# snarkify/sirius

Hardware: AMD Instinct MI355X
Metric: IVC fold-steps/s (CycleFold IVC::next hot path, Poseidon-shaped synthetic trace, 2^k rows) (higher is better)
Workload: dtype u256 (modular; 9 x 29-bit / 8 x 32-bit limbs)

## Files before the change

sirius_amd/csrc/msm.h:

```cpp
#pragma once
#include "curve.cuh"
#include "devrt.h"
#include "glv.cuh"
#include "stripes.h"
#include "tuning.h"

#include <cstdlib>

namespace srs {
namespace msm {

constexpr int WBITS = 16;
constexpr int NWIN = 16;
constexpr int NWIN_COMPACT = 8;
constexpr uint32_t PAY_ENDO = 1u << 30;
constexpr uint32_t NBUCKET = 1u << (WBITS - 1);

constexpr uint32_t SORT_THREADS = 1024;
constexpr uint32_t SORT_TILE_MIN = 8192;
constexpr uint32_t SORT_TARGET_BLOCKS = 256;
constexpr uint32_t SEG = 128, SEG_BUCKETS = NBUCKET / SEG;
constexpr uint32_t SORT_TILE2 = 8192;
constexpr uint64_t TWO_PASS_MIN_SLOTS = 1ull << 23;
constexpr uint32_t PLAN_THREADS = 1024;
constexpr uint32_t ACC_THREADS = 256;
constexpr uint32_t ACC_L0_LOG = 4, ACC_L0 = 1u << ACC_L0_LOG;
constexpr uint32_t ACC_L1_LOG = 3, ACC_L1 = 1u << ACC_L1_LOG;
constexpr uint32_t FINAL_THREADS = 256;
constexpr uint32_t FINAL_FANIN = 512;
constexpr int MAX_LEVELS = 8;
constexpr uint32_t RED_ROWS = 256;
constexpr uint32_t RED_COLS = NBUCKET / RED_ROWS;
constexpr uint32_t RED_THREADS = 4 * RED_COLS;
constexpr uint32_t ACC1_QUAD_MAX = 1u << 17;
constexpr uint32_t BATCH_ARGS = 16;
constexpr uint32_t LANDING_SLOTS = 16;
constexpr uint32_t NORM_G = 16;
constexpr uint32_t SLOT_LOG = 6;
constexpr uint32_t SLOT_L0_MIN_LOG = 2, SLOT_L0_MAX_LOG = 16;
constexpr int WBITS_W = 20;
constexpr int NWIN_W = 13;
constexpr uint32_t NSEG_W = 16;
constexpr uint32_t WIDE_THREADS = 256, WIDE_PER = 2, WIDE_TILE = WIDE_THREADS * WIDE_PER;
constexpr uint32_t WIDE_MIN_KEY_LOG = 23;
constexpr uint32_t WIDE_MIN_N_LOG = 23;

static_assert(RED_ROWS == 256 && RED_COLS == 128, "k_rowcol lane layout");
static_assert(NBUCKET % PLAN_THREADS == 0, "k_plan tiling");

inline bool expect_ovf_initial() { return tuning::get_or(tuning::MSM_EXPECT_OVF, 1) != 0; }

struct Key {
    int curve = 0;
    size_t len = 0;
    size_t global_len = 0;
    uint32_t rank = 0, world = 1;
    bool compact = false;
    bool compact_scalars = false;
    affine_t *table = nullptr;
    affine_t *table_w = nullptr;
    uint64_t stat_slot_sets = 0, stat_hot_sets = 0, stat_redo = 0, stat_other_sets = 0;
    uint64_t last_entries = 0;
    uint64_t last_scalars = 0;

    Arena arena;
    void *h_result = nullptr;
    struct Landing { bool wide = false, slot_mode = false, ovf_on = false; uint32_t batch = 0; } landing[LANDING_SLOTS];
    xyzz_t *fold_buckets = nullptr;
    xyzz_t *slots = nullptr;
    size_t slots_pts = 0;
    uint8_t *used = nullptr;
    uint32_t *h_ovf = nullptr;
    uint32_t slot_s = 0;
    uint32_t seq = 0;
    bool commit_ovf = false;
    bool expect_ovf = expect_ovf_initial();
    uint32_t cold_streak = 0;
};

int choose_windows(Key &k);
void build_table(Key &k, hipStream_t stream);
size_t table_bytes(const Key &k);
void release(Key &k);
void generate_bases(Key &k, uint64_t seed, hipStream_t stream);

void read_bases(const Key &k, affine_t *out_dev, hipStream_t stream);

size_t count_off_curve(const Key &k, hipStream_t stream);

size_t workspace_bytes(uint32_t n_max, uint32_t batch);

void run(Key &k, const fe_t *const *scalars_dev, const uint32_t *n_host, uint32_t batch, int is_mont,
         hipStream_t stream, xyzz_t *result_host);

enum Fold { FOLD_NONE = 0, FOLD_FIRST = 1, FOLD_MIDDLE = 2, FOLD_LAST = 3 };
bool enqueue(Key &k, const fe_t *const *scalars_dev, const uint32_t *n_host, const uint32_t *base_host, uint32_t batch, int is_mont,
             hipStream_t stream, uint32_t slot, Fold fold = FOLD_NONE);
void finish(Key &k, uint32_t batch, uint32_t slot, bool launched, xyzz_t *result_host);
void reserve(Key &k, uint32_t n_max, uint32_t batch);
bool overflow_missed(const Key &k, uint32_t slot);
void note_commit(Key &k, const uint32_t *slots_used, uint32_t n_slots, uint64_t scalars);

}
}
```

sirius_amd/csrc/msm.hip:

```cpp
#define SRS_F29_CHAIN 1
#include "msm.h"
#include "tuning.h"
#include "curve29.cuh"
#include "prof.h"

#include <algorithm>
#include <cstdlib>
#include <numeric>
#include <vector>

namespace srs {
namespace msm {

__device__ __forceinline__ uint32_t upper_bucket(const uint32_t *__restrict__ tp, uint32_t t) {
    uint32_t lo = 0, hi = NBUCKET;
    while (hi - lo > 1) {
        uint32_t mid = (lo + hi) >> 1;
        if (tp[mid] <= t) lo = mid; else hi = mid;
    }
    return lo;
}

template <class C>
__global__ void k_table_step(const affine_t *__restrict__ prev, xyzz_t *__restrict__ tmp, uint32_t n, int nbits) {
    uint32_t i = blockIdx.x * blockDim.x + threadIdx.x;
    if (i >= n) return;
    affine_t p = prev[i];
    xyzz_t a;
    if (Ec<C>::is_identity(p)) {
        a = Ec<C>::identity();
    } else {
        a = Ec<C>::dbl_affine(p);
        for (int k = 1; k < nbits; ++k) a = Ec<C>::dbl(a);
    }
    tmp[i] = a;
}

template <class C>
__global__ void k_normalize(const xyzz_t *__restrict__ in, affine_t *__restrict__ out, uint32_t n) {
    using F = typename C::F;
    uint32_t g = blockIdx.x * blockDim.x + threadIdx.x;
    size_t lo = (size_t)g * NORM_G;
    if (lo >= n) return;
    uint32_t cnt = (uint32_t)((n - lo < NORM_G) ? (n - lo) : NORM_G);
    fe_t pre[NORM_G];
    fe_t acc = F::one();
    for (uint32_t j = 0; j < cnt; ++j) {
        pre[j] = acc;
        xyzz_t p = in[lo + j];
        if (!Ec<C>::is_identity(p)) acc = F::mul(acc, F::mul(p.zz, p.zzz));
    }
    fe_t inv = F::inv(acc);
    for (uint32_t j = cnt; j-- > 0;) {
        xyzz_t p = in[lo + j];
        affine_t o;
        if (Ec<C>::is_identity(p)) {
            o = Ec<C>::affine_identity();
        } else {
            fe_t i = F::mul(inv, pre[j]);
            inv = F::mul(inv, F::mul(p.zz, p.zzz));
            o.x = F::mul(p.x, F::mul(i, p.zzz));
            o.y = F::mul(p.y, F::mul(i, p.zz));
        }
        out[lo + j] = o;
    }
}

template <class C>
__global__ void k_table_form(affine_t *__restrict__ t, size_t n) {
    size_t i = (size_t)blockIdx.x * blockDim.x + threadIdx.x;
    if (i >= n) return;
    t[i] = Ec29<C>::table_form(t[i]);
}
template <class C>
__device__ __forceinline__ affine_t table_unform(const affine_t &q) {
    using G = typename C::F;
    fe_t c = G::one();
    for (int d = 0; d < 5; ++d) c = G::halve(c);
    affine_t o;
    o.x = G::mul(q.x, c);
    o.y = G::mul(q.y, c);
    return o;
}
template <class C>
__global__ void k_table_unform(const affine_t *__restrict__ t, affine_t *__restrict__ out, size_t n) {
    size_t i = (size_t)blockIdx.x * blockDim.x + threadIdx.x;
    if (i >= n) return;
    out[i] = table_unform<C>(t[i]);
}

__device__ __forceinline__ uint64_t splitmix64(uint64_t &s) {
    uint64_t z = (s += 0x9e3779b97f4a7c15ull);
    z = (z ^ (z >> 30)) * 0xbf58476d1ce4e5b9ull;
    z = (z ^ (z >> 27)) * 0x94d049bb133111ebull;
    return z ^ (z >> 31);
}
template <class C>
__global__ void k_gen_bases(xyzz_t *__restrict__ tmp, uint32_t n, uint64_t seed, uint32_t rank, uint32_t world) {
    using F = typename C::F;
    uint32_t i = blockIdx.x * blockDim.x + threadIdx.x;
    if (i >= n) return;
    uint64_t g = Stripes{rank, world}.global_index((size_t)i);
    uint64_t st = seed ^ (g * 0x100000001b3ull + 0xcbf29ce484222325ull);
    uint32_t k[8];
    for (int j = 0; j < 4; ++j) {
        uint64_t v = splitmix64(st);
        k[2 * j] = (uint32_t)v;
        k[2 * j + 1] = (uint32_t)(v >> 32);
    }
    k[7] &= 0x0FFFFFFFu;
    k[0] |= 1u;
    affine_t gen;
    gen.x = F::one();
    if (C::ID == 0) {
        gen.y = F::dbl(F::one());
    } else {
        fe_t y;
        const uint32_t yc[8] = {0x823f272cu, 0x833fc48du, 0xf1181294u, 0x2d270d45u, 0x06a45d63u, 0xcf135e75u, 0x00000002u, 0u};
        for (int j = 0; j < 8; ++j) y.v[j] = yc[j];
        gen.y = F::to_mont(y);
    }
    tmp[i] = Ec<C>::mul_canon(k, gen);
}

template <class C>
__global__ void k_on_curve(const affine_t *__restrict__ pts, uint32_t n, uint32_t *__restrict__ bad) {
    uint32_t i = blockIdx.x * blockDim.x + threadIdx.x;
    if (i >= n) return;
    if (!Ec<C>::is_on_curve(table_unform<C>(pts[i]))) atomicAdd(bad, 1u);
}

struct BatchDesc {
    const fe_t *ptr[BATCH_ARGS];
    uint32_t n[BATCH_ARGS];
    uint32_t base[BATCH_ARGS];
};

__device__ __forceinline__ void recode_half(const uint32_t (&k)[4], bool neg, uint16_t *__restrict__ d, size_t n) {
    const uint32_t top = neg ? 0x7FFFu : 0x8000u;
    uint32_t carry = 0;
#pragma unroll
    for (int w = 0; w < NWIN_COMPACT; ++w) {
        const uint32_t v = ((k[w >> 1] >> ((w & 1) * 16)) & 0xFFFFu) + carry;
        const bool borrow = v > top;
        const uint32_t mag = borrow ? 0x10000u - v : v;
        const bool minus = borrow != neg;
        carry = borrow ? 1u : 0u;
        d[(size_t)w * n] = (uint16_t)(mag ? ((mag - 1u) | (minus ? 0x8000u : 0u)) : 0xFFFFu);
    }
}

template <class C, bool COMPACT>
__global__ void k_digits(BatchDesc bd, uint16_t *__restrict__ dig, size_t dig_stride, int is_mont, uint32_t rank, uint32_t world,
                         uint32_t *__restrict__ count_zero, uint32_t n_zero) {
    using S = typename C::S;
    uint32_t m = blockIdx.y;
    uint32_t n = bd.n[m];
    uint32_t i = blockIdx.x * blockDim.x + threadIdx.x;
    for (uint32_t j = (blockIdx.y * gridDim.x + blockIdx.x) * blockDim.x + threadIdx.x; j < n_zero; j += gridDim.x * gridDim.y * blockDim.x)
        count_zero[j] = 0;
    if (i >= n) return;
    fe_t s = bd.ptr[m][Stripes{rank, world}.global_index((size_t)i)];
    if (is_mont) s = S::from_mont(s);
    uint16_t *d = dig + (size_t)m * dig_stride;
    if (COMPACT) {
        const glv_t g = glv_decompose<C>(s);
        recode_half(g.k1, g.neg1, d + i, n);
        recode_half(g.k2, g.neg2, d + (size_t)NWIN_COMPACT * n + i, n);
        return;
    }
    uint32_t carry = 0;
#pragma unroll
    for (int w = 0; w < NWIN; ++w) {
        uint32_t raw = (s.v[w >> 1] >> ((w & 1) * 16)) & 0xFFFFu;
        uint32_t v = raw + carry;
        uint32_t code;
        if (v > 0x8000u) {
            code = ((0x10000u - v) - 1u) | 0x8000u;
            carry = 1;
        } else {
            code = v ? (v - 1u) : 0xFFFFu;
            carry = 0;
        }
        d[(size_t)w * n + i] = (uint16_t)code;
    }
}

template <class Fn>
__device__ __forceinline__ void for_each_digit(const uint16_t *__restrict__ d, uint32_t lo, uint32_t hi, Fn fn) {
    uint32_t head = lo;
    while (head < hi && (reinterpret_cast<uintptr_t>(d + head) & 15u)) ++head;
    for (uint32_t i = lo + threadIdx.x; i < head; i += blockDim.x) fn(i, (uint32_t)d[i]);
    const uint32_t nvec = (hi - head) / 8;
    const uint4 *v = reinterpret_cast<const uint4 *>(d + head);
    auto eight = [&](uint32_t q, const uint4 &x) {
        const uint32_t i0 = head + q * 8;
        fn(i0 + 0, x.x & 0xFFFFu); fn(i0 + 1, x.x >> 16);
        fn(i0 + 2, x.y & 0xFFFFu); fn(i0 + 3, x.y >> 16);
        fn(i0 + 4, x.z & 0xFFFFu); fn(i0 + 5, x.z >> 16);
        fn(i0 + 6, x.w & 0xFFFFu); fn(i0 + 7, x.w >> 16);
    };
    uint32_t q = threadIdx.x;
    for (; q + 3 * blockDim.x < nvec; q += 4 * blockDim.x) {
        const uint4 x0 = v[q], x1 = v[q + blockDim.x], x2 = v[q + 2 * blockDim.x], x3 = v[q + 3 * blockDim.x];
        eight(q, x0); eight(q + blockDim.x, x1); eight(q + 2 * blockDim.x, x2); eight(q + 3 * blockDim.x, x3);
    }
    for (; q < nvec; q += blockDim.x) eight(q, v[q]);
    for (uint32_t i = head + nvec * 8 + threadIdx.x; i < hi; i += blockDim.x) fn(i, (uint32_t)d[i]);
}

__device__ __forceinline__ void tile_histogram(uint32_t *h, const uint16_t *__restrict__ d, uint32_t lo, uint32_t hi) {
    for (uint32_t b = threadIdx.x; b < NBUCKET; b += blockDim.x) h[b] = 0;
    __syncthreads();
    for_each_digit(d, lo, hi, [&](uint32_t, uint32_t code) {
        if (code != 0xFFFFu) atomicAdd(&h[code & 0x7FFFu], 1u);
    });
    __syncthreads();
}

__global__ void SRS_KERNEL_BOUNDS(SORT_THREADS, 1)
    k_hist(const uint16_t *__restrict__ dig, size_t dig_stride, BatchDesc bd,
           uint32_t *__restrict__ count , uint32_t SORT_TILE,
           uint32_t *__restrict__ tile_hist ) {
    __shared__ uint32_t h[NBUCKET];
    uint32_t m = blockIdx.z, w = blockIdx.y;
    uint32_t n = bd.n[m];
    uint32_t lo = blockIdx.x * SORT_TILE;
    const uint32_t T1 = gridDim.x * NWIN, t1 = w * gridDim.x + blockIdx.x;
    if (lo >= n) {
        if (tile_hist)
            for (uint32_t sgm = threadIdx.x; sgm < SEG; sgm += blockDim.x) tile_hist[((size_t)m * SEG + sgm) * T1 + t1] = 0;
        return;
    }
    uint32_t hi = lo + SORT_TILE < n ? lo + SORT_TILE : n;
    const uint16_t *d = dig + (size_t)m * dig_stride + (size_t)w * n;
    tile_histogram(h, d, lo, hi);
    uint32_t *cnt = count + (size_t)m * NBUCKET;
    const uint32_t rot = ((blockIdx.y * gridDim.x + blockIdx.x) * 128u) & (NBUCKET - 1);
    for (uint32_t i = threadIdx.x; i < NBUCKET; i += blockDim.x) {
        const uint32_t b = (i + rot) & (NBUCKET - 1);
        uint32_t c = h[b];
        if (c) atomicAdd(&cnt[b], c);
    }
    if (tile_hist) {
        for (uint32_t sgm = threadIdx.x; sgm < SEG; sgm += blockDim.x) {
            uint32_t c = 0;
            for (uint32_t b = 0; b < SEG_BUCKETS; ++b) c += h[sgm * SEG_BUCKETS + ((b + sgm) & (SEG_BUCKETS - 1))];
            tile_hist[((size_t)m * SEG + sgm) * T1 + t1] = c;
        }
    }
}

__device__ __forceinline__ uint32_t block_exclusive_scan(uint32_t v, uint32_t *lds, uint32_t *total);

__global__ void SRS_KERNEL_BOUNDS(1024, 1)
    k_scan_seg(uint32_t *__restrict__ tile_hist, uint32_t T1, const uint32_t *__restrict__ plan, size_t plan_stride) {
    __shared__ uint32_t lds[64];
    const uint32_t sgm = blockIdx.x, m = blockIdx.y;
    uint32_t *row = tile_hist + ((size_t)m * SEG + sgm) * T1;
    const uint32_t base = plan[(size_t)m * plan_stride + (size_t)sgm * SEG_BUCKETS];
    uint32_t carry = 0;
    for (uint32_t at = 0; at < T1; at += blockDim.x) {
        const uint32_t i = at + threadIdx.x;
        const uint32_t v = i < T1 ? row[i] : 0;
        uint32_t total;
        const uint32_t ex = block_exclusive_scan(v, lds, &total);
        if (i < T1) row[i] = base + carry + ex;
        carry += total;
    }
}

constexpr uint32_t GRP_PER = 16, GRP_SUB = SORT_THREADS * GRP_PER;
template <bool COMPACT>
__device__ __forceinline__ uint32_t payload_base(uint32_t w, uint32_t table_stride, uint32_t base) {
    if (COMPACT) return ((w & (NWIN_COMPACT - 1)) * table_stride + base) | (w >= NWIN_COMPACT ? PAY_ENDO : 0u);
    return w * table_stride + base;
}
template <bool COMPACT>
__global__ void SRS_KERNEL_BOUNDS(SORT_THREADS, 1)
    k_group(const uint16_t *__restrict__ dig, size_t dig_stride, BatchDesc bd, const uint32_t *__restrict__ tile_hist,
            uint16_t *__restrict__ gkey, uint32_t *__restrict__ gpay, size_t g_stride, uint32_t table_stride, uint32_t SORT_TILE,
            const uint32_t *__restrict__ plan, size_t plan_stride, uint16_t *__restrict__ tb, size_t tb_stride, uint32_t arr) {
    __shared__ uint32_t cur[SEG], cnt[SEG], lb[SEG], sc[64];
    __shared__ uint32_t spay[GRP_SUB];
    __shared__ uint16_t skey[GRP_SUB];
    const uint32_t m = blockIdx.z, w = blockIdx.y, tid = threadIdx.x;
    if (tb) {
        const uint32_t *tp = plan + (size_t)m * plan_stride + (size_t)arr * (NBUCKET + 1);
        uint16_t *map = tb + (size_t)m * tb_stride;
        const uint32_t waves = gridDim.x * gridDim.y * (blockDim.x >> 6);
        const uint32_t wv = (blockIdx.y * gridDim.x + blockIdx.x) * (blockDim.x >> 6) + (tid >> 6), lane = tid & 63u;
        for (uint32_t b = wv; b < NBUCKET; b += waves) {
            const uint32_t s = tp[b], e = tp[b + 1];
            for (uint32_t t = s + lane; t < e; t += 64) map[t] = (uint16_t)b;
        }
    }
    const uint32_t n = bd.n[m];
    const uint32_t lo = blockIdx.x * SORT_TILE;
    if (lo >= n) return;
    const uint32_t hi = lo + SORT_TILE < n ? lo + SORT_TILE : n;
    const uint32_t T1 = gridDim.x * NWIN, t1 = w * gridDim.x + blockIdx.x;
    for (uint32_t sgm = tid; sgm < SEG; sgm += blockDim.x) cur[sgm] = tile_hist[((size_t)m * SEG + sgm) * T1 + t1];
    const uint16_t *d = dig + (size_t)m * dig_stride + (size_t)w * n;
    uint16_t *ok = gkey + (size_t)m * g_stride;
    uint32_t *op = gpay + (size_t)m * g_stride;
    const uint32_t pay0 = payload_base<COMPACT>(w, table_stride, bd.base[m]);
    for (uint32_t sub = lo; sub < hi; sub += GRP_SUB) {
        for (uint32_t sgm = tid; sgm < SEG; sgm += blockDim.x) cnt[sgm] = 0;
        __syncthreads();
        const uint32_t i0 = sub + tid * GRP_PER;
        uint32_t code[GRP_PER], rank[GRP_PER];
        if (i0 + GRP_PER <= hi && (reinterpret_cast<uintptr_t>(d + i0) & 15u) == 0) {
            const uint4 *v = reinterpret_cast<const uint4 *>(d + i0);
#pragma unroll
            for (uint32_t q = 0; q < GRP_PER / 8; ++q) {
                const uint4 x = v[q];
                code[8 * q + 0] = x.x & 0xFFFFu; code[8 * q + 1] = x.x >> 16;
                code[8 * q + 2] = x.y & 0xFFFFu; code[8 * q + 3] = x.y >> 16;
                code[8 * q + 4] = x.z & 0xFFFFu; code[8 * q + 5] = x.z >> 16;
                code[8 * q + 6] = x.w & 0xFFFFu; code[8 * q + 7] = x.w >> 16;
            }
        } else {
#pragma unroll
            for (uint32_t k = 0; k < GRP_PER; ++k) code[k] = i0 + k < hi ? (uint32_t)d[i0 + k] : 0xFFFFu;
        }
#pragma unroll
        for (uint32_t k = 0; k < GRP_PER; ++k)
            rank[k] = code[k] != 0xFFFFu ? atomicAdd(&cnt[(code[k] & 0x7FFFu) / SEG_BUCKETS], 1u) : 0u;
        __syncthreads();
        uint32_t n_sub;
        const uint32_t ex = block_exclusive_scan(tid < SEG ? cnt[tid] : 0u, sc, &n_sub);
        if (tid < SEG) lb[tid] = ex;
        __syncthreads();
#pragma unroll
        for (uint32_t k = 0; k < GRP_PER; ++k) {
            if (code[k] != 0xFFFFu) {
                const uint32_t bkt = code[k] & 0x7FFFu, pos = lb[bkt / SEG_BUCKETS] + rank[k];
                skey[pos] = (uint16_t)bkt;
                spay[pos] = (pay0 + i0 + k) | ((code[k] & 0x8000u) << 16);
            }
        }
        __syncthreads();
        for (uint32_t i = tid; i < n_sub; i += blockDim.x) {
            const uint32_t key = skey[i], sgm = key / SEG_BUCKETS, g = cur[sgm] + (i - lb[sgm]);
            ok[g] = (uint16_t)key;
            op[g] = spay[i];
        }
        __syncthreads();
        if (tid < SEG) cur[tid] += cnt[tid];
    }
}

constexpr uint32_t S2_PER = 8, S2_RANGE = 2 * SEG_BUCKETS;
static_assert(SORT_TILE2 == SORT_THREADS * S2_PER, "k_scatter2: one tile = S2_PER entries per thread");
__global__ void SRS_KERNEL_BOUNDS(SORT_THREADS, 2)
    k_scatter2(const uint16_t *__restrict__ gkey, const uint32_t *__restrict__ gpay, size_t g_stride,
               const uint32_t *__restrict__ plan, size_t plan_stride, uint32_t *__restrict__ cursor ,
               uint32_t *__restrict__ sorted, size_t sorted_stride, uint32_t TILE2) {
    __shared__ uint32_t cnt[S2_RANGE], lb[S2_RANGE], gb[S2_RANGE], sc[64];
    __shared__ uint32_t spay[SORT_TILE2];
    __shared__ uint16_t skey[SORT_TILE2];
    const uint32_t m = blockIdx.y, tid = threadIdx.x;
    const uint32_t total = plan[(size_t)m * plan_stride + NBUCKET];
    const uint32_t n_tiles = (total + TILE2 - 1) / TILE2, per_xcd = (n_tiles + 7) / 8;
    if (blockIdx.x / 8 >= per_xcd) return;
    const uint32_t tile_id = (blockIdx.x % 8) * per_xcd + blockIdx.x / 8;
    if (tile_id >= n_tiles) return;
    const uint32_t lo = tile_id * TILE2;
    if (lo >= total) return;
    const uint32_t hi = lo + TILE2 < total ? lo + TILE2 : total;
    const uint16_t *key = gkey + (size_t)m * g_stride;
    const uint32_t *pay = gpay + (size_t)m * g_stride;
    uint32_t *cur = cursor + (size_t)m * NBUCKET;
    uint32_t *out = sorted + (size_t)m * sorted_stride;
    const uint32_t b_lo = ((uint32_t)key[lo] / SEG_BUCKETS) * SEG_BUCKETS;
    const uint32_t b_hi = ((uint32_t)key[hi - 1] / SEG_BUCKETS + 1) * SEG_BUCKETS;
    if (b_hi - b_lo > S2_RANGE) {
        for (uint32_t i = lo + tid; i < hi; i += blockDim.x) out[atomicAdd(&cur[key[i]], 1u)] = pay[i];
        return;
    }
    for (uint32_t b = tid; b < S2_RANGE; b += blockDim.x) cnt[b] = 0;
    __syncthreads();
    const uint32_t i0 = lo + tid * S2_PER;
    uint32_t kk[S2_PER], pp[S2_PER], rank[S2_PER];
    if (i0 + S2_PER <= hi && (reinterpret_cast<uintptr_t>(key + i0) & 15u) == 0 && (reinterpret_cast<uintptr_t>(pay + i0) & 15u) == 0) {
        const uint4 x = *reinterpret_cast<const uint4 *>(key + i0);
        kk[0] = x.x & 0xFFFFu; kk[1] = x.x >> 16; kk[2] = x.y & 0xFFFFu; kk[3] = x.y >> 16;
        kk[4] = x.z & 0xFFFFu; kk[5] = x.z >> 16; kk[6] = x.w & 0xFFFFu; kk[7] = x.w >> 16;
        const uint4 p0 = *reinterpret_cast<const uint4 *>(pay + i0), p1 = *reinterpret_cast<const uint4 *>(pay + i0 + 4);
        pp[0] = p0.x; pp[1] = p0.y; pp[2] = p0.z; pp[3] = p0.w; pp[4] = p1.x; pp[5] = p1.y; pp[6] = p1.z; pp[7] = p1.w;
    } else {
#pragma unroll
        for (uint32_t k = 0; k < S2_PER; ++k) {
            kk[k] = i0 + k < hi ? (uint32_t)key[i0 + k] : 0xFFFFu;
            pp[k] = i0 + k < hi ? pay[i0 + k] : 0u;
        }
    }
#pragma unroll
    for (uint32_t k = 0; k < S2_PER; ++k) rank[k] = kk[k] != 0xFFFFu ? atomicAdd(&cnt[kk[k] - b_lo], 1u) : 0u;
    __syncthreads();
    uint32_t n_tile;
    const uint32_t c = tid < S2_RANGE ? cnt[tid] : 0u;
    const uint32_t ex = block_exclusive_scan(c, sc, &n_tile);
    if (tid < S2_RANGE) {
        lb[tid] = ex;
        gb[tid] = c ? atomicAdd(&cur[b_lo + tid], c) : 0u;
    }
    __syncthreads();
#pragma unroll
    for (uint32_t k = 0; k < S2_PER; ++k) {
        if (kk[k] != 0xFFFFu) {
            const uint32_t pos = lb[kk[k] - b_lo] + rank[k];
            skey[pos] = (uint16_t)(kk[k] - b_lo);
            spay[pos] = pp[k];
        }
    }
    __syncthreads();
    for (uint32_t i = tid; i < n_tile; i += blockDim.x) {
        const uint32_t b = skey[i];
        out[gb[b] + (i - lb[b])] = spay[i];
    }
}

#ifndef SCATTER_RES_INFLIGHT
#define SCATTER_RES_INFLIGHT 4
#endif
template <bool COMPACT>
__global__ void SRS_KERNEL_BOUNDS(SORT_THREADS, 1)
    k_scatter(const uint16_t *__restrict__ dig, size_t dig_stride, BatchDesc bd,
              uint32_t *__restrict__ cursor , uint32_t *__restrict__ sorted,
              size_t sorted_stride, uint32_t table_stride, uint32_t SORT_TILE) {
    __shared__ uint32_t h[NBUCKET];
    uint32_t m = blockIdx.z, w = blockIdx.y;
    uint32_t n = bd.n[m];
    uint32_t lo = blockIdx.x * SORT_TILE;
    if (lo >= n) return;
    uint32_t hi = lo + SORT_TILE < n ? lo + SORT_TILE : n;
    const uint16_t *d = dig + (size_t)m * dig_stride + (size_t)w * n;
    tile_histogram(h, d, lo, hi);
    uint32_t *cur = cursor + (size_t)m * NBUCKET;
    constexpr int RES = SCATTER_RES_INFLIGHT;
    for (uint32_t b0 = threadIdx.x; b0 < NBUCKET; b0 += RES * blockDim.x) {
        uint32_t c[RES], r[RES];
#pragma unroll
        for (int u = 0; u < RES; ++u) c[u] = b0 + u * blockDim.x < NBUCKET ? h[b0 + u * blockDim.x] : 0u;
#pragma unroll
        for (int u = 0; u < RES; ++u) r[u] = c[u] ? atomicAdd(&cur[b0 + u * blockDim.x], c[u]) : 0u;
#pragma unroll
        for (int u = 0; u < RES; ++u) if (c[u]) h[b0 + u * blockDim.x] = r[u];
    }
    __syncthreads();
    uint32_t *out = sorted + (size_t)m * sorted_stride;
    const uint32_t pay0 = payload_base<COMPACT>(w, table_stride, bd.base[m]);
    for_each_digit(d, lo, hi, [&](uint32_t i, uint32_t code) {
        if (code != 0xFFFFu) {
            uint32_t pos = atomicAdd(&h[code & 0x7FFFu], 1u);
            out[pos] = (pay0 + i) | ((code & 0x8000u) << 16);
        }
    });
}

struct Link {
    uint32_t base[MAX_LEVELS + 1][NSEG_W + 1];
};
__device__ __forceinline__ uint32_t link_segment(const uint32_t *__restrict__ base, uint32_t t) {
    uint32_t v = 0;
#pragma unroll
    for (uint32_t u = 1; u < NSEG_W; ++u) v += (t >= base[u]) ? 1u : 0u;
    return v;
}

struct WideDesc {
    const fe_t *ptr;
    uint32_t n, base;
    uint32_t rank, world;
    int is_mont;
};

template <class C>
__device__ __forceinline__ void wide_codes(const WideDesc &wd, uint32_t i, uint32_t (&code)[NWIN_W]) {
    using S = typename C::S;
    if (i >= wd.n) {
#pragma unroll
        for (int w = 0; w < NWIN_W; ++w) code[w] = 0xFFFFFFFFu;
        return;
    }
    fe_t s = wd.ptr[Stripes{wd.rank, wd.world}.global_index((size_t)i)];
    if (wd.is_mont) s = S::from_mont(s);
    uint32_t carry = 0;
#pragma unroll
    for (int w = 0; w < NWIN_W; ++w) {
        const int bit = WBITS_W * w, limb = bit >> 5, sh = bit & 31;
        uint64_t two = s.v[limb];
        if (limb + 1 < 8) two |= (uint64_t)s.v[limb + 1] << 32;
        const uint32_t v = ((uint32_t)(two >> sh) & 0xFFFFFu) + carry;
        if (v > 0x80000u) {
            code[w] = ((0x100000u - v) - 1u) | 0x80000000u;
            carry = 1;
        } else {
            code[w] = v ? (v - 1u) : 0xFFFFFFFFu;
            carry = 0;
        }
    }
}

template <class C, bool GROUP>
__global__ void SRS_KERNEL_BOUNDS(WIDE_THREADS, 1)
    k_seg_pass(WideDesc wd, uint32_t *__restrict__ tile_cnt, uint32_t T, uint32_t *__restrict__ seg_total,
               uint16_t *__restrict__ gkey, uint32_t *__restrict__ gpay, uint32_t table_stride) {
    constexpr uint32_t NW = WIDE_THREADS / 64, STAGE = GROUP ? WIDE_TILE * NWIN_W : 1;
    __shared__ uint32_t wc[NW][NSEG_W];
    __shared__ uint32_t ss[NSEG_W + 1], goff[NSEG_W];
    __shared__ uint16_t skey[STAGE];
    __shared__ uint32_t spay[STAGE];
    const uint32_t tile = blockIdx.x, wave = threadIdx.x >> 6;
    if (threadIdx.x < NW * NSEG_W) (&wc[0][0])[threadIdx.x] = 0;
    uint32_t code[WIDE_PER][NWIN_W];
#pragma unroll
    for (uint32_t k = 0; k < WIDE_PER; ++k) wide_codes<C>(wd, tile * WIDE_TILE + k * WIDE_THREADS + threadIdx.x, code[k]);
    __syncthreads();
#pragma unroll
    for (uint32_t k = 0; k < WIDE_PER; ++k) {
#pragma unroll
        for (int w = 0; w < NWIN_W; ++w) {
            const uint32_t c = code[k][w];
            if (c != 0xFFFFFFFFu) atomicAdd(&wc[wave][(c >> 15) & (NSEG_W - 1)], 1u);
        }
    }
    __syncthreads();
    if (threadIdx.x < NSEG_W) {
        const uint32_t v = threadIdx.x;
        uint32_t tot = 0;
        for (uint32_t w = 0; w < NW; ++w) tot += wc[w][v];
        if (!GROUP) {
            tile_cnt[(size_t)v * T + tile] = tot;
            if (tot) atomicAdd(&seg_total[v], tot);
        } else {
            ss[v + 1] = tot;
            goff[v] = tile_cnt[(size_t)v * T + tile];
        }
    }
    if (!GROUP) return;
    __syncthreads();
    if (threadIdx.x == 0) {
        uint32_t run = 0;
        for (uint32_t v = 0; v < NSEG_W; ++v) {
            const uint32_t c = ss[v + 1];
            ss[v] = run;
            run += c;
        }
        ss[NSEG_W] = run;
    }
    __syncthreads();
    if (threadIdx.x < NSEG_W) {
        const uint32_t v = threadIdx.x;
        uint32_t run = ss[v];
        for (uint32_t w = 0; w < NW; ++w) {
            const uint32_t c = wc[w][v];
            wc[w][v] = run;
            run += c;
        }
    }
    __syncthreads();
#pragma unroll
    for (uint32_t k = 0; k < WIDE_PER; ++k) {
        const uint32_t i = tile * WIDE_TILE + k * WIDE_THREADS + threadIdx.x;
#pragma unroll
        for (int w = 0; w < NWIN_W; ++w) {
            const uint32_t c = code[k][w];
            if (c != 0xFFFFFFFFu) {
                const uint32_t pos = atomicAdd(&wc[wave][(c >> 15) & (NSEG_W - 1)], 1u);
                skey[pos] = (uint16_t)(c & 0x7FFFu);
                spay[pos] = ((uint32_t)w * table_stride + wd.base + i) | (c & 0x80000000u);
            }
        }
    }
    __syncthreads();
    for (uint32_t v = 0; v < NSEG_W; ++v) {
        const uint32_t lo = ss[v], hi = ss[v + 1], g0 = goff[v];
        for (uint32_t e = lo + threadIdx.x; e < hi; e += WIDE_THREADS) {
            gkey[g0 + (e - lo)] = skey[e];
            gpay[g0 + (e - lo)] = spay[e];
        }
    }
}

__global__ void SRS_KERNEL_BOUNDS(1024, 1)
    k_seg_scan(uint32_t *__restrict__ tile_cnt, uint32_t T, const uint32_t *__restrict__ seg_total, uint32_t *__restrict__ seg_off,
               uint32_t *__restrict__ tile_base ,
               uint32_t *__restrict__ tile_base2 ,
               uint32_t small_tiles ) {
    __shared__ uint32_t lds[64];
    const uint32_t v = blockIdx.x;
    uint32_t base = 0;
    for (uint32_t u = 0; u < v; ++u) base += seg_total[u];
    if (v == 0 && threadIdx.x == 0) {
        uint32_t all = 0;
        for (uint32_t u = 0; u < NSEG_W; ++u) all += seg_total[u];
        uint32_t tile_g = (all + (SORT_TARGET_BLOCKS - NSEG_W) - 1) / (SORT_TARGET_BLOCKS - NSEG_W);
        tile_g = (tile_g + 1023u) & ~1023u;
        if (tile_g < SORT_TILE_MIN) tile_g = SORT_TILE_MIN;
        tile_base[NSEG_W + 1] = tile_g;
        uint32_t run = 0, tr = 0;
        for (uint32_t u = 0; u < NSEG_W; ++u) {
            seg_off[u] = run;
            tile_base[u] = tr;
            run += seg_total[u];
            tr += (seg_total[u] + tile_g - 1) / tile_g;
        }
        seg_off[NSEG_W] = run;
        tile_base[NSEG_W] = tr;
        const uint32_t tile2 = (small_tiles && all / (NSEG_W * NBUCKET) < 40u) ? SORT_TILE2 / 4 : SORT_TILE2;
        uint32_t t2 = 0;
        for (uint32_t u = 0; u < NSEG_W; ++u) {
            tile_base2[u] = t2;
            t2 += (seg_total[u] + tile2 - 1) / tile2;
        }
        tile_base2[NSEG_W] = t2;
        tile_base2[NSEG_W + 1] = tile2;
    }
    uint32_t *row = tile_cnt + (size_t)v * T;
    uint32_t carry = 0;
    for (uint32_t at = 0; at < T; at += blockDim.x) {
        const uint32_t i = at + threadIdx.x;
        const uint32_t c = i < T ? row[i] : 0;
        uint32_t total;
        const uint32_t ex = block_exclusive_scan(c, lds, &total);
        if (i < T) row[i] = base + carry + ex;
        carry += total;
    }
}

__device__ __forceinline__ bool wide_tile(const uint32_t *__restrict__ seg_off, const uint32_t *__restrict__ tile_base,
                                          uint32_t &v, uint32_t &lo, uint32_t &hi) {
    if (blockIdx.x >= tile_base[NSEG_W]) return false;
    const uint32_t tile_g = tile_base[NSEG_W + 1];
    v = link_segment(tile_base, blockIdx.x);
    lo = seg_off[v] + (blockIdx.x - tile_base[v]) * tile_g;
    hi = seg_off[v + 1];
    if (hi > lo + tile_g) hi = lo + tile_g;
    return true;
}

__global__ void SRS_KERNEL_BOUNDS(SORT_THREADS, 1)
    k_hist_g(const uint16_t *__restrict__ gkey, const uint32_t *__restrict__ seg_off, const uint32_t *__restrict__ tile_base,
             uint32_t *__restrict__ count , uint32_t *__restrict__ tile_hist ) {
    __shared__ uint32_t h[NBUCKET];
    uint32_t v, lo, hi;
    if (!wide_tile(seg_off, tile_base, v, lo, hi)) return;
    tile_histogram(h, gkey, lo, hi);
    uint32_t *cnt = count + (size_t)v * NBUCKET;
    for (uint32_t b = threadIdx.x; b < NBUCKET; b += blockDim.x) {
        uint32_t c = h[b];
        if (c) atomicAdd(&cnt[b], c);
    }
    if (tile_hist) {
        for (uint32_t sgm = threadIdx.x; sgm < SEG; sgm += blockDim.x) {
            uint32_t c = 0;
            for (uint32_t b = 0; b < SEG_BUCKETS; ++b) c += h[sgm * SEG_BUCKETS + ((b + sgm) & (SEG_BUCKETS - 1))];
            tile_hist[(size_t)sgm * gridDim.x + blockIdx.x] = c;
        }
    }
}

__global__ void SRS_KERNEL_BOUNDS(1024, 1)
    k_scan_seg_g(uint32_t *__restrict__ tile_hist, uint32_t TG, const uint32_t *__restrict__ tile_base, const uint32_t *__restrict__ plan,
                 size_t plan_stride) {
    __shared__ uint32_t lds[64];
    const uint32_t sgm = blockIdx.x, v = blockIdx.y;
    const uint32_t t0 = tile_base[v], t1 = tile_base[v + 1];
    uint32_t *row = tile_hist + (size_t)sgm * TG;
    const uint32_t base = plan[(size_t)v * plan_stride + (size_t)sgm * SEG_BUCKETS];
    uint32_t carry = 0;
    for (uint32_t at = t0; at < t1; at += blockDim.x) {
        const uint32_t i = at + threadIdx.x;
        const uint32_t c = i < t1 ? row[i] : 0;
        uint32_t total;
        const uint32_t ex = block_exclusive_scan(c, lds, &total);
        if (i < t1) row[i] = base + carry + ex;
        carry += total;
    }
}

__global__ void SRS_KERNEL_BOUNDS(SORT_THREADS, 1)
    k_group_g(const uint16_t *__restrict__ gkey, const uint32_t *__restrict__ gpay, const uint32_t *__restrict__ seg_off,
              const uint32_t *__restrict__ tile_base, const uint32_t *__restrict__ tile_hist, uint16_t *__restrict__ gkey2,
              uint32_t *__restrict__ gpay2) {
    __shared__ uint32_t cur[SEG], cnt[SEG], lb[SEG], sc[64];
    __shared__ uint32_t spay[GRP_SUB];
    __shared__ uint16_t skey[GRP_SUB];
    const uint32_t tid = threadIdx.x;
    uint32_t v, lo, hi;
    if (!wide_tile(seg_off, tile_base, v, lo, hi)) return;
    for (uint32_t sgm = tid; sgm < SEG; sgm += blockDim.x) cur[sgm] = tile_hist[(size_t)sgm * gridDim.x + blockIdx.x];
    for (uint32_t sub = lo; sub < hi; sub += GRP_SUB) {
        for (uint32_t sgm = tid; sgm < SEG; sgm += blockDim.x) cnt[sgm] = 0;
        __syncthreads();
        uint32_t key[GRP_PER], pay[GRP_PER], rank[GRP_PER];
#pragma unroll
        for (uint32_t k = 0; k < GRP_PER; ++k) {
            const uint32_t i = sub + k * SORT_THREADS + tid;
            key[k] = i < hi ? (uint32_t)gkey[i] : 0xFFFFu;
            pay[k] = i < hi ? gpay[i] : 0u;
        }
#pragma unroll
        for (uint32_t k = 0; k < GRP_PER; ++k) rank[k] = key[k] != 0xFFFFu ? atomicAdd(&cnt[key[k] / SEG_BUCKETS], 1u) : 0u;
        __syncthreads();
        uint32_t n_sub;
        const uint32_t ex = block_exclusive_scan(tid < SEG ? cnt[tid] : 0u, sc, &n_sub);
        if (tid < SEG) lb[tid] = ex;
        __syncthreads();
#pragma unroll
        for (uint32_t k = 0; k < GRP_PER; ++k) {
            if (key[k] != 0xFFFFu) {
                const uint32_t pos = lb[key[k] / SEG_BUCKETS] + rank[k];
                skey[pos] = (uint16_t)key[k];
                spay[pos] = pay[k];
            }
        }
        __syncthreads();
        for (uint32_t i = tid; i < n_sub; i += blockDim.x) {
            const uint32_t kk = skey[i], sgm = kk / SEG_BUCKETS, g = cur[sgm] + (i - lb[sgm]);
            gkey2[g] = (uint16_t)kk;
            gpay2[g] = spay[i];
        }
        __syncthreads();
        if (tid < SEG) cur[tid] += cnt[tid];
    }
}

__global__ void SRS_KERNEL_BOUNDS(SORT_THREADS, 2)
    k_scatter2_g(const uint16_t *__restrict__ gkey2, const uint32_t *__restrict__ gpay2, const uint32_t *__restrict__ seg_off,
                 const uint32_t *__restrict__ tile_base2, uint32_t *__restrict__ cursor ,
                 uint32_t *__restrict__ sorted) {
    __shared__ uint32_t cnt[S2_RANGE], lb[S2_RANGE], gb[S2_RANGE], sc[64];
    __shared__ uint32_t spay[SORT_TILE2];
    __shared__ uint16_t skey[SORT_TILE2];
    const uint32_t tid = threadIdx.x;
    const uint32_t n_tiles = tile_base2[NSEG_W], per_xcd = (n_tiles + 7) / 8;
    if (blockIdx.x / 8 >= per_xcd) return;
    const uint32_t tile_id = (blockIdx.x % 8) * per_xcd + blockIdx.x / 8;
    if (tile_id >= n_tiles) return;
    const uint32_t v = link_segment(tile_base2, tile_id), tile2 = tile_base2[NSEG_W + 1];
    const uint32_t lo = seg_off[v] + (tile_id - tile_base2[v]) * tile2;
    const uint32_t hi = lo + tile2 < seg_off[v + 1] ? lo + tile2 : seg_off[v + 1];
    if (lo >= hi) return;
    uint32_t *cur = cursor + (size_t)v * NBUCKET;
    const uint32_t b_lo = ((uint32_t)gkey2[lo] / SEG_BUCKETS) * SEG_BUCKETS;
    const uint32_t b_hi = ((uint32_t)gkey2[hi - 1] / SEG_BUCKETS + 1) * SEG_BUCKETS;
    if (b_hi - b_lo > S2_RANGE) {
        for (uint32_t i = lo + tid; i < hi; i += blockDim.x) sorted[atomicAdd(&cur[gkey2[i]], 1u)] = gpay2[i];
        return;
    }
    for (uint32_t b = tid; b < S2_RANGE; b += blockDim.x) cnt[b] = 0;
    __syncthreads();
    uint32_t kk[S2_PER], pp[S2_PER], rank[S2_PER];
#pragma unroll
    for (uint32_t k = 0; k < S2_PER; ++k) {
        const uint32_t i = lo + k * SORT_THREADS + tid;
        kk[k] = i < hi ? (uint32_t)gkey2[i] : 0xFFFFu;
        pp[k] = i < hi ? gpay2[i] : 0u;
    }
#pragma unroll
    for (uint32_t k = 0; k < S2_PER; ++k) rank[k] = kk[k] != 0xFFFFu ? atomicAdd(&cnt[kk[k] - b_lo], 1u) : 0u;
    __syncthreads();
    uint32_t n_tile;
    const uint32_t c = tid < S2_RANGE ? cnt[tid] : 0u;
    const uint32_t ex = block_exclusive_scan(c, sc, &n_tile);
    if (tid < S2_RANGE) {
        lb[tid] = ex;
        gb[tid] = c ? atomicAdd(&cur[b_lo + tid], c) : 0u;
    }
    __syncthreads();
#pragma unroll
    for (uint32_t k = 0; k < S2_PER; ++k) {
        if (kk[k] != 0xFFFFu) {
            const uint32_t pos = lb[kk[k] - b_lo] + rank[k];
            skey[pos] = (uint16_t)(kk[k] - b_lo);
            spay[pos] = pp[k];
        }
    }
    __syncthreads();
    for (uint32_t i = tid; i < n_tile; i += blockDim.x) {
        const uint32_t b = skey[i];
        sorted[gb[b] + (i - lb[b])] = spay[i];
    }
}

__device__ __forceinline__ uint32_t block_exclusive_scan(uint32_t v, uint32_t *lds, uint32_t *total) {
    const uint32_t t = threadIdx.x, lane = t & 63u, wave = t >> 6, nwaves = blockDim.x >> 6;
    uint32_t x = v;
#pragma unroll
    for (uint32_t d = 1; d < 64; d <<= 1) {
        uint32_t y = __shfl_up(x, d, 64);
        if (lane >= d) x += y;
    }
    if (lane == 63) lds[wave] = x;
    __syncthreads();
    if (wave == 0) {
        uint32_t w = lane < nwaves ? lds[lane] : 0;
#pragma unroll
        for (uint32_t d = 1; d < 64; d <<= 1) {
            uint32_t y = __shfl_up(w, d, 64);
            if (lane >= d) w += y;
        }
        if (lane < nwaves) lds[lane] = w;
    }
    __syncthreads();
    uint32_t base = wave ? lds[wave - 1] : 0;
    *total = lds[nwaves - 1];
    __syncthreads();
    return base + x - v;
}

__device__ __forceinline__ uint32_t block_max(uint32_t v, uint32_t *lds) {
    const uint32_t t = threadIdx.x, lane = t & 63u, wave = t >> 6, nwaves = blockDim.x >> 6;
#pragma unroll
    for (uint32_t d = 32; d >= 1; d >>= 1) {
        uint32_t y = __shfl_xor(v, d, 64);
        v = y > v ? y : v;
    }
    if (lane == 0) lds[wave] = v;
    __syncthreads();
    uint32_t m = 0;
    for (uint32_t w = 0; w < nwaves; ++w) m = lds[w] > m ? lds[w] : m;
    __syncthreads();
    return m;
}

__global__ void SRS_KERNEL_BOUNDS(PLAN_THREADS, 1)
    k_plan(const uint32_t *__restrict__ count, uint32_t *__restrict__ cursor, uint32_t *__restrict__ plan,
           size_t plan_stride, int nlevels, uint32_t l0_log, uint32_t l1_log,
           const uint32_t *__restrict__ seg_off ) {
    constexpr uint32_t PER = NBUCKET / PLAN_THREADS;
    __shared__ uint32_t tile[NBUCKET + NBUCKET / PER];
    __shared__ uint32_t lds[64];
    const uint32_t t = threadIdx.x;
    const uint32_t m = blockIdx.x;
    const int my_level = (int)blockIdx.y - 1;
    const uint32_t *cnt = count + (size_t)m * NBUCKET;
    uint32_t *cur = cursor + (size_t)m * NBUCKET;
    uint32_t *pl = plan + (size_t)m * plan_stride;
    {
        uint32_t c[PER];
#pragma unroll
        for (uint32_t j = 0; j < PER; ++j) c[j] = cnt[t + j * PLAN_THREADS];
#pragma unroll
        for (uint32_t j = 0; j < PER; ++j) {
            const uint32_t i = t + j * PLAN_THREADS;
            tile[i + i / PER] = c[j];
        }
    }
    __syncthreads();
    const uint32_t base = t * PER + t;
    auto value = [&](uint32_t c, int level) -> uint32_t {
        uint32_t p = (c + (1u << l0_log) - 1) >> l0_log;
        p = p ? p : 1u;
        for (int l = 0; l < level; ++l) p = (p + (1u << l1_log) - 1) >> l1_log;
        return p;
    };
    uint32_t local = 0;
#pragma unroll 8
    for (uint32_t j = 0; j < PER; ++j) local += tile[base + j];
    uint32_t total_entries;
    uint32_t run = block_exclusive_scan(local, lds, &total_entries);
    uint32_t total = total_entries;
    int needed = nlevels;
    if (my_level >= 0) {
        uint32_t mx = 0;
#pragma unroll 8
        for (uint32_t j = 0; j < PER; ++j) {
            const uint32_t v = value(tile[base + j], 0);
            mx = v > mx ? v : mx;
        }
        uint32_t p = block_max(mx, lds);
        needed = 1;
        while (p > FINAL_FANIN && needed < nlevels) {
            p = (p + (1u << l1_log) - 1) >> l1_log;
            ++needed;
        }
        const uint32_t typical = (2u * total_entries + NBUCKET - 1) / NBUCKET;
        uint32_t x = (typical + (1u << l0_log) - 1) >> l0_log;
        int by_mean = 1;
        while (x > 1 && by_mean < nlevels) {
            x = (x + (1u << l1_log) - 1) >> l1_log;
            ++by_mean;
        }
        needed = by_mean > needed ? by_mean : needed;
        if (t == 0 && my_level == 0) pl[plan_stride - 4] = (uint32_t)needed;
        if (my_level >= needed) return;
        local = 0;
#pragma unroll 8
        for (uint32_t j = 0; j < PER; ++j) local += value(tile[base + j], my_level);
        run = block_exclusive_scan(local, lds, &total);
    }
    uint32_t mx_own = 0;
#pragma unroll 8
    for (uint32_t j = 0; j < PER; ++j) {
        const uint32_t c = tile[base + j], v = my_level < 0 ? c : value(c, my_level);
        tile[base + j] = run;
        run += v;
        mx_own = v > mx_own ? v : mx_own;
    }
    __syncthreads();
    uint32_t *o = pl + (size_t)(my_level + 1) * (NBUCKET + 1);
    const uint32_t shift = (my_level < 0 && seg_off) ? seg_off[m] : 0u;
    for (uint32_t i = t; i < NBUCKET; i += PLAN_THREADS) {
        const uint32_t v = tile[i + i / PER] + shift;
        o[i] = v;
        if (my_level < 0) cur[i] = v;
    }
    if (t == PLAN_THREADS - 1) o[NBUCKET] = total + shift;
    if (my_level == needed - 1) {
        const uint32_t p = block_max(mx_own, lds);
        if (t == 0) pl[plan_stride - 3] = (p <= 1u) ? 1u : 0u;
    }
}

__device__ __forceinline__ uint32_t slot_l0_log(uint32_t total_entries, uint32_t S, uint32_t want_cap) {
    const uint32_t mean = total_entries / NBUCKET;
    uint32_t r = 0;
    while ((r + 1) * (r + 1) <= mean) ++r;
    const uint32_t thresh = mean + 6 * r + 1;
    uint32_t lg = SLOT_L0_MIN_LOG;
    while (((thresh + (1u << lg) - 1) >> lg) > S - 1 && lg < SLOT_L0_MAX_LOG) ++lg;
    uint32_t want = 0;
    while (want < want_cap && (total_entries >> (19 + want + 1)) != 0) ++want;
    return lg > want ? lg : want;
}

__global__ void SRS_KERNEL_BOUNDS(PLAN_THREADS, 1)
    k_plan_s(const uint32_t *__restrict__ count, uint32_t *__restrict__ cursor, uint32_t *__restrict__ plan, size_t plan_stride, int nlevels,
             uint32_t S, uint32_t l1_log, const uint8_t *__restrict__ used_prev, uint8_t *__restrict__ used_next, int first,
             uint32_t *__restrict__ h_ovf, uint32_t want_cap) {
    constexpr uint32_t PER = NBUCKET / PLAN_THREADS;
    __shared__ uint32_t tile[NBUCKET + NBUCKET / PER];
    __shared__ uint32_t lds[64];
    const uint32_t t = threadIdx.x, m = blockIdx.x, role = blockIdx.y;
    const uint32_t *cnt = count + (size_t)m * NBUCKET;
    uint32_t *pl = plan + (size_t)m * plan_stride;
    {
        uint32_t c[PER];
#pragma unroll
        for (uint32_t j = 0; j < PER; ++j) c[j] = cnt[t + j * PLAN_THREADS];
#pragma unroll
        for (uint32_t j = 0; j < PER; ++j) {
            const uint32_t i = t + j * PLAN_THREADS;
            tile[i + i / PER] = c[j];
        }
    }
    __syncthreads();
    const uint32_t base = t * PER + t;
    uint32_t local = 0;
#pragma unroll 8
    for (uint32_t j = 0; j < PER; ++j) local += tile[base + j];
    uint32_t total_entries;
    uint32_t run = block_exclusive_scan(local, lds, &total_entries);
    const uint32_t l0_log = slot_l0_log(total_entries, S, want_cap);
    uint32_t total = total_entries;
    const bool dense = role == (uint32_t)nlevels + 1;
    const uint32_t lv = role >= 2 && !dense ? role - 1 : 0;
    auto value = [&](uint32_t c) -> uint32_t {
        if (role == 0) return c;
        uint32_t p = (c + (1u << l0_log) - 1) >> l0_log;
        if (dense) return p;
        p = p > S - 1 ? p - (S - 1) : 0u;
        for (uint32_t l = 0; l < lv; ++l) p = (p + (1u << l1_log) - 1) >> l1_log;
        return p;
    };
    if (role != 0) {
        local = 0;
        uint32_t mx = 0;
#pragma unroll 4
        for (uint32_t j = 0; j < PER; ++j) {
            const uint32_t c = tile[base + j];
            local += value(c);
            if (!dense) {
                const uint32_t p = (c + (1u << l0_log) - 1) >> l0_log, o = p > S - 1 ? p - (S - 1) : 0u;
                mx = o > mx ? o : mx;
            }
        }
        if (!dense) {
            uint32_t p = block_max(mx, lds);
            int needed = 1;
            while (p > FINAL_FANIN && needed < nlevels) {
                p = (p + (1u << l1_log) - 1) >> l1_log;
                ++needed;
            }
            if (role == 1 && t == 0) {
                pl[plan_stride - 4] = (uint32_t)needed;
                pl[plan_stride - 3] = 0;
                pl[plan_stride - 2] = l0_log;
            }
            if ((int)role - 1 >= needed) return;
        }
        run = block_exclusive_scan(local, lds, &total);
    }
    static_assert(PER == 32, "k_plan_s: used[] travels as 2 x uint4 per thread");
    uint32_t was_w[8] = {0, 0, 0, 0, 0, 0, 0, 0}, now_w[8] = {0, 0, 0, 0, 0, 0, 0, 0};
    if (dense && !first) {
        const uint4 *up = reinterpret_cast<const uint4 *>(used_prev + (size_t)m * NBUCKET + (size_t)t * PER);
        const uint4 a = up[0], b = up[1];
        was_w[0] = a.x; was_w[1] = a.y; was_w[2] = a.z; was_w[3] = a.w; was_w[4] = b.x; was_w[5] = b.y; was_w[6] = b.z; was_w[7] = b.w;
    }
#pragma unroll
    for (uint32_t j = 0; j < PER; ++j) {
        const uint32_t c = tile[base + j], v = value(c);
        tile[base + j] = run;
        run += v;
        if (dense) {
            const uint32_t now = v < S - 1 ? v : S - 1, was = (was_w[j >> 2] >> (8 * (j & 3))) & 0xFFu;
            now_w[j >> 2] |= (now > was ? now : was) << (8 * (j & 3));
        }
    }
    if (dense) {
        uint4 *un = reinterpret_cast<uint4 *>(used_next + (size_t)m * NBUCKET + (size_t)t * PER);
        uint4 lo, hi;
        lo.x = now_w[0]; lo.y = now_w[1]; lo.z = now_w[2]; lo.w = now_w[3];
        hi.x = now_w[4]; hi.y = now_w[5]; hi.z = now_w[6]; hi.w = now_w[7];
        un[0] = lo;
        un[1] = hi;
    }
    __syncthreads();
    uint32_t *o = pl + (size_t)role * (NBUCKET + 1);
    uint32_t *cur = cursor + (size_t)m * NBUCKET;
    for (uint32_t i = t; i < NBUCKET; i += PLAN_THREADS) {
        const uint32_t v = tile[i + i / PER];
        o[i] = v;
        if (role == 0) cur[i] = v;
    }
    if (t == PLAN_THREADS - 1) {
        o[NBUCKET] = total;
        if (role == 1) {
            pl[plan_stride - 1] = total;
            h_ovf[m] = total;
        }
        if (role == 0) h_ovf[(size_t)LANDING_SLOTS * BATCH_ARGS + m] = total;
    }
}

__global__ void k_link(const uint32_t *__restrict__ plan, size_t plan_stride, int nlevels, Link *__restrict__ link) {
    const uint32_t t = threadIdx.x;
    for (int l = 0; l < nlevels; ++l) {
        uint32_t c = 0;
        if (t < NSEG_W) {
            const uint32_t *pl = plan + (size_t)t * plan_stride;
            if ((uint32_t)l < pl[plan_stride - 4]) c = pl[(size_t)(l + 1) * (NBUCKET + 1) + NBUCKET];
        }
        uint32_t x = c;
#pragma unroll
        for (uint32_t d = 1; d < NSEG_W; d <<= 1) {
            uint32_t y = __shfl_up(x, d, 64);
            if (t >= d) x += y;
        }
        if (t < NSEG_W) link->base[l][t] = x - c;
        if (t == NSEG_W - 1) link->base[l][NSEG_W] = x;
    }
}

__global__ void SRS_KERNEL_BOUNDS(256, 1)
    k_expand(const uint32_t *__restrict__ plan, size_t plan_stride, uint16_t *__restrict__ tb, size_t tb_stride,
             const Link *__restrict__ link, uint32_t arr ) {
    const uint32_t m = blockIdx.y, lane = threadIdx.x & 63u;
    const uint32_t b = blockIdx.x * 4 + (threadIdx.x >> 6);
    const uint32_t *tp = plan + (size_t)m * plan_stride + (size_t)arr * (NBUCKET + 1);
    uint16_t *out = tb + (link ? (size_t)link->base[0][m] : (size_t)m * tb_stride);
    const uint32_t s = tp[b], e = tp[b + 1];
    for (uint32_t t = s + lane; t < e; t += 64) out[t] = (uint16_t)b;
}

template <class C, bool COMPACT>
__device__ __forceinline__ aff29_t load_entry(const affine_t &p, uint32_t v) {
    aff29_t q = Ec29<C>::load_raw(p);
    if (COMPACT) {
        if (v & PAY_ENDO) {
            f29_t beta;
#pragma unroll
            for (int i = 0; i < 9; ++i) beta.v[i] = GlvConsts<C::ID>::beta29(i);
            q.x = Ec29<C>::F::mul(q.x, beta);
        }
    }
    return q;
}
template <bool COMPACT>
__device__ __forceinline__ uint32_t entry_index(uint32_t v) { return v & (COMPACT ? PAY_ENDO - 1u : 0x7FFFFFFFu); }

template <class C, bool COMPACT>
__device__ __forceinline__ xyzz29_t accumulate_part(const uint32_t *__restrict__ src, uint32_t s, uint32_t e, const affine_t *__restrict__ table,
                                                    const xyzz_t *__restrict__ init) {
    using E29 = Ec29<C>;
    using F = typename E29::F;
    bool exc = false;
    xyzz29_t acc;
    {
        uint32_t v = src[s];
        uint32_t vn = s + 1 < e ? src[s + 1] : 0u;
        affine_t p = table[entry_index<COMPACT>(v)];
        uint32_t j = s;
        if (init) {
            acc = E29::unpack(*init);
        } else {
            affine_t pn = p;
            uint32_t vnn = 0;
            if (s + 1 < e) {
                pn = table[entry_index<COMPACT>(vn)];
                if (s + 2 < e) vnn = src[s + 2];
            }
            const aff29_t q = load_entry<C, COMPACT>(p, v);
            acc.x = q.x;
            acc.y = (v >> 31) ? F::normalize(F::template neg_lazy<1, 0>(q.y)) : q.y;
            acc.zz = E29::one();
            acc.zzz = acc.zz;
            exc = F::is_zero_exact(q.y);
            v = vn;
            vn = vnn;
            p = pn;
            j = s + 1;
        }
        for (; j < e; ++j) {
            uint32_t vnn = 0;
            affine_t pn = p;
            if (j + 1 < e) {
                pn = table[entry_index<COMPACT>(vn)];
                if (j + 2 < e) vnn = src[j + 2];
            }
            acc = E29::madd_signed_fast(acc, load_entry<C, COMPACT>(p, v), (v >> 31) != 0, exc);
            v = vn;
            vn = vnn;
            p = pn;
        }
    }
    if (exc) {
        acc = init ? E29::unpack(*init) : E29::identity();
#pragma unroll 1
        for (uint32_t j = s; j < e; ++j) {
            const uint32_t v = src[j];
            acc = E29::madd_signed(acc, load_entry<C, COMPACT>(table[entry_index<COMPACT>(v)], v), (v >> 31) != 0);
        }
    }
    return acc;
}

template <class C, bool COMPACT>
__device__ __forceinline__ void accum0_thread(const uint32_t *__restrict__ sorted, size_t sorted_stride, const uint32_t *__restrict__ plan,
                                              size_t plan_stride, const uint16_t *__restrict__ tb, size_t tb_stride,
                                              const affine_t *__restrict__ table, xyzz_t *__restrict__ parts, size_t parts_stride, uint32_t l0,
                                              const Link *__restrict__ link) {
    uint32_t m = blockIdx.y;
    uint32_t t = blockIdx.x * blockDim.x + threadIdx.x;
    size_t slot;
    if (link) {
        if (t >= link->base[0][NSEG_W]) return;
        m = link_segment(link->base[0], t);
        slot = t;
        t -= link->base[0][m];
    } else {
        slot = (size_t)m * parts_stride + t;
    }
    const uint32_t *off = plan + (size_t)m * plan_stride;
    const uint32_t *tp = off + (NBUCKET + 1);
    if (t >= tp[NBUCKET]) return;
    uint32_t b = tb[link ? slot : (size_t)m * tb_stride + t];
    uint32_t part = t - tp[b];
    uint32_t s = off[b] + part * l0;
    uint32_t e = off[b + 1];
    if (e > s + l0) e = s + l0;
    const uint32_t *src = link ? sorted : sorted + (size_t)m * sorted_stride;
    using E29 = Ec29<C>;
    const xyzz29_t acc = s < e ? accumulate_part<C, COMPACT>(src, s, e, table, nullptr) : E29::identity();
    parts[slot] = E29::pack(acc);
}
template <class C>
__global__ void SRS_KERNEL_BOUNDS(ACC_THREADS, 1)
    k_accum0(const uint32_t *__restrict__ sorted, size_t sorted_stride, const uint32_t *__restrict__ plan,
             size_t plan_stride, const uint16_t *__restrict__ tb, size_t tb_stride, const affine_t *__restrict__ table,
             xyzz_t *__restrict__ parts, size_t parts_stride, uint32_t l0, const Link *__restrict__ link) {
    accum0_thread<C, false>(sorted, sorted_stride, plan, plan_stride, tb, tb_stride, table, parts, parts_stride, l0, link);
}
template <class C>
__global__ void SRS_KERNEL_BOUNDS(ACC_THREADS, 1)
    k_accum0c(const uint32_t *__restrict__ sorted, size_t sorted_stride, const uint32_t *__restrict__ plan,
              size_t plan_stride, const uint16_t *__restrict__ tb, size_t tb_stride, const affine_t *__restrict__ table,
              xyzz_t *__restrict__ parts, size_t parts_stride, uint32_t l0, const Link *__restrict__ link) {
    accum0_thread<C, true>(sorted, sorted_stride, plan, plan_stride, tb, tb_stride, table, parts, parts_stride, l0, link);
}

__device__ __forceinline__ xyzz_t shfl_down_point(const xyzz_t &p, unsigned delta) {
    xyzz_t o;
    shfl_down_words<32>(reinterpret_cast<const uint32_t *>(&p), reinterpret_cast<uint32_t *>(&o), delta, 64);
    return o;
}

__device__ __forceinline__ xyzz29_t shfl_down_point29(const xyzz29_t &p, unsigned delta, int width) {
    xyzz29_t o;
    shfl_down_words<36>(reinterpret_cast<const uint32_t *>(&p), reinterpret_cast<uint32_t *>(&o), delta, width);
    return o;
}

template <class C>
__global__ void SRS_KERNEL_BOUNDS(ACC_THREADS, 1)
    k_accum1(const xyzz_t *__restrict__ in, size_t in_stride, const uint32_t *__restrict__ plan,
             size_t plan_stride, int level, xyzz_t *__restrict__ out, size_t out_stride, uint32_t l1,
             const Link *__restrict__ link, uint32_t quad_max) {
    uint32_t m = blockIdx.y;
    const uint32_t lin = blockIdx.x * blockDim.x + threadIdx.x;
    uint32_t t;
    bool quad;
    size_t in_off, out_off;
    if (link) {
        const uint32_t n_all = link->base[level][NSEG_W];
        quad = n_all <= quad_max;
        t = quad ? (lin >> 2) : lin;
        if (t >= n_all) return;
        m = link_segment(link->base[level], t);
        t -= link->base[level][m];
        in_off = link->base[(level - 1) & 1][m];
        out_off = link->base[level & 1][m];
    } else {
        in_off = (size_t)m * in_stride;
        out_off = (size_t)m * out_stride;
    }
    if ((uint32_t)level >= plan[(size_t)m * plan_stride + plan_stride - 4]) return;
    const uint32_t *tp_prev = plan + (size_t)m * plan_stride + (size_t)level * (NBUCKET + 1);
    const uint32_t *tp = tp_prev + (NBUCKET + 1);
    const uint32_t n_out = tp[NBUCKET];
    if (!link) {
        quad = (uint64_t)n_out * gridDim.y <= quad_max;
        t = quad ? (lin >> 2) : lin;
    }
    if (t >= n_out) return;
    uint32_t b = upper_bucket(tp, t);
    uint32_t part = t - tp[b];
    uint32_t s = tp_prev[b] + part * l1;
    uint32_t e = tp_prev[b + 1];
    if (e > s + l1) e = s + l1;
    using E29 = Ec29<C>;
    const xyzz_t *src = in + in_off;
    xyzz29_t acc = E29::unpack(src[s]);
    if (quad) {
        const uint32_t q = threadIdx.x & 3u;
        for (uint32_t j = s + 1; j < e; ++j) acc = E29::add_quad(acc, E29::unpack(src[j]), q);
        if (q == 0) out[out_off + t] = E29::pack(acc);
    } else {
        for (uint32_t j = s + 1; j < e; ++j) acc = E29::add(acc, E29::unpack(src[j]));
        out[out_off + t] = E29::pack(acc);
    }
}

template <class C>
__global__ void SRS_KERNEL_BOUNDS(FINAL_THREADS, 1)
    k_accum_final(const xyzz_t *__restrict__ ping, size_t ping_stride, const xyzz_t *__restrict__ pong,
                  size_t pong_stride, const uint32_t *__restrict__ plan, size_t plan_stride,
                  xyzz_t *__restrict__ buckets, const Link *__restrict__ link) {
    uint32_t m = blockIdx.y;
    if (plan[(size_t)m * plan_stride + plan_stride - 3]) return;
    const uint32_t level = plan[(size_t)m * plan_stride + plan_stride - 4];
    const xyzz_t *in = (level & 1u) ? ping : pong;
    const size_t in_stride = (level & 1u) ? ping_stride : pong_stride;
    const uint32_t *tp = plan + (size_t)m * plan_stride + (size_t)level * (NBUCKET + 1);
    uint32_t lane = threadIdx.x & 63u;
    uint32_t b = blockIdx.x * (blockDim.x >> 6) + (threadIdx.x >> 6);
    uint32_t s = tp[b], e = tp[b + 1];
    const xyzz_t *src = in + (link ? (size_t)link->base[(level - 1u) & 1u][m] : (size_t)m * in_stride);
    xyzz_t *dst = buckets + (size_t)m * NBUCKET;
    if (e - s == 1) {
        if (lane == 0) dst[b] = src[s];
        return;
    }
    using E29 = Ec29<C>;
    xyzz29_t acc = E29::identity();
    for (uint32_t j = s + lane; j < e; j += 64) acc = E29::add(acc, E29::unpack(src[j]));
    for (unsigned d = 32; d >= 1; d >>= 1) {
        xyzz29_t other = shfl_down_point29(acc, d, 64);
        if (lane < d) acc = E29::add(acc, other);
    }
    if (lane == 0) dst[b] = E29::pack(acc);
}

template <class C, bool COMPACT>
__device__ __forceinline__ void accum0s_thread(const uint32_t *__restrict__ sorted, size_t sorted_stride, const uint32_t *__restrict__ plan,
                                               size_t plan_stride, uint32_t arr, const uint16_t *__restrict__ tb, size_t tb_stride,
                                               const affine_t *__restrict__ table, xyzz_t *__restrict__ slots, uint32_t S,
                                               const uint8_t *__restrict__ used_prev, int first, xyzz_t *__restrict__ ovf, size_t ovf_stride) {
    const uint32_t m = blockIdx.y;
    const uint32_t t = blockIdx.x * blockDim.x + threadIdx.x;
    const uint32_t *off = plan + (size_t)m * plan_stride;
    const uint32_t *tp = off + (size_t)arr * (NBUCKET + 1);
    if (t >= tp[NBUCKET]) return;
    const uint32_t *tpo = off + (NBUCKET + 1);
    const uint32_t l0 = 1u << off[plan_stride - 2];
    const uint32_t b = tb[(size_t)m * tb_stride + t];
    const uint32_t part = t - tp[b];
    uint32_t s = off[b] + part * l0;
    uint32_t e = off[b + 1];
    if (e > s + l0) e = s + l0;
    const uint32_t *src = sorted + (size_t)m * sorted_stride;
    using E29 = Ec29<C>;
    const bool regular = part < S - 1;
    xyzz_t *slot = regular ? slots + ((size_t)m * NBUCKET + b) * S + part : ovf + (size_t)m * ovf_stride + tpo[b] + (part - (S - 1));
    const bool resume = regular && !first && part < (uint32_t)used_prev[(size_t)m * NBUCKET + b];
    *slot = E29::pack(accumulate_part<C, COMPACT>(src, s, e, table, resume ? slot : nullptr));
}
template <class C>
__global__ void SRS_KERNEL_BOUNDS(ACC_THREADS, 1)
    k_accum0s(const uint32_t *__restrict__ sorted, size_t sorted_stride, const uint32_t *__restrict__ plan, size_t plan_stride, uint32_t arr,
              const uint16_t *__restrict__ tb, size_t tb_stride, const affine_t *__restrict__ table, xyzz_t *__restrict__ slots, uint32_t S,
              const uint8_t *__restrict__ used_prev, int first, xyzz_t *__restrict__ ovf, size_t ovf_stride) {
    accum0s_thread<C, false>(sorted, sorted_stride, plan, plan_stride, arr, tb, tb_stride, table, slots, S, used_prev, first, ovf, ovf_stride);
}
template <class C>
__global__ void SRS_KERNEL_BOUNDS(ACC_THREADS, 1)
    k_accum0sc(const uint32_t *__restrict__ sorted, size_t sorted_stride, const uint32_t *__restrict__ plan, size_t plan_stride, uint32_t arr,
               const uint16_t *__restrict__ tb, size_t tb_stride, const affine_t *__restrict__ table, xyzz_t *__restrict__ slots, uint32_t S,
               const uint8_t *__restrict__ used_prev, int first, xyzz_t *__restrict__ ovf, size_t ovf_stride) {
    accum0s_thread<C, true>(sorted, sorted_stride, plan, plan_stride, arr, tb, tb_stride, table, slots, S, used_prev, first, ovf, ovf_stride);
}

template <class C>
__global__ void SRS_KERNEL_BOUNDS(FINAL_THREADS, 1)
    k_ovf_final(const xyzz_t *__restrict__ ping, size_t ping_stride, const xyzz_t *__restrict__ pong, size_t pong_stride,
                const uint32_t *__restrict__ plan, size_t plan_stride, xyzz_t *__restrict__ slots, uint32_t S, int first) {
    const uint32_t m = blockIdx.y;
    const uint32_t level = plan[(size_t)m * plan_stride + plan_stride - 4];
    const xyzz_t *in = (level & 1u) ? ping + (size_t)m * ping_stride : pong + (size_t)m * pong_stride;
    const uint32_t *tp = plan + (size_t)m * plan_stride + (size_t)level * (NBUCKET + 1);
    const uint32_t lane = threadIdx.x & 63u;
    const uint32_t b = blockIdx.x * (blockDim.x >> 6) + (threadIdx.x >> 6);
    const uint32_t s = tp[b], e = tp[b + 1];
    xyzz_t *dst = slots + ((size_t)m * NBUCKET + b) * S + (S - 1);
    using E29 = Ec29<C>;
    if (e == s) {
        if (first && lane == 0) *dst = E29::pack(E29::identity());
        return;
    }
    xyzz29_t acc = E29::identity();
    for (uint32_t j = s + lane; j < e; j += 64) acc = E29::add(acc, E29::unpack(in[j]));
    for (unsigned d = 32; d >= 1; d >>= 1) {
        xyzz29_t other = shfl_down_point29(acc, d, 64);
        if (lane < d) acc = E29::add(acc, other);
    }
    if (lane == 0) {
        if (!first) acc = E29::add(acc, E29::unpack(*dst));
        *dst = E29::pack(acc);
    }
}

template <class C, bool QUAD>
__global__ void SRS_KERNEL_BOUNDS(256, 1)
    k_slot_reduce(const xyzz_t *__restrict__ in, uint32_t in_pb, const uint8_t *__restrict__ used, size_t used_stride, int extra,
                  xyzz_t *__restrict__ out, uint32_t out_pb) {
    using E29 = Ec29<C>;
    const uint32_t m = blockIdx.y;
    const uint32_t lin = blockIdx.x * blockDim.x + threadIdx.x, t = QUAD ? (lin >> 2) : lin, q = lin & 3u;
    if (t >= NBUCKET * out_pb) return;
    const uint32_t g = t / NBUCKET, b = t % NBUCKET;
    const uint32_t lim = used ? (uint32_t)used[(size_t)m * used_stride + b] : in_pb;
    const xyzz_t *src = in + ((size_t)m * NBUCKET + b) * in_pb;
    xyzz29_t acc = E29::identity();
    for (uint32_t idx = g; idx < in_pb; idx += out_pb) {
        if (!(idx < lim || (int)idx == extra)) continue;
        const xyzz29_t x = E29::unpack(src[idx]);
        if (QUAD) acc = E29::add_quad(acc, x, q); else acc = E29::add(acc, x);
    }
    if (!QUAD || q == 0) out[((size_t)m * NBUCKET + b) * out_pb + g] = E29::pack(acc);
}

template <class C>
__global__ void SRS_KERNEL_BOUNDS(64, 1)
    k_bucket_fold(const xyzz_t *__restrict__ buckets, const xyzz_t *__restrict__ ping, const xyzz_t *__restrict__ pong,
                  const uint32_t *__restrict__ plan, size_t plan_stride, xyzz_t *__restrict__ total, int first) {
    using E29 = Ec29<C>;
    const uint32_t b = blockIdx.x * blockDim.x + threadIdx.x;
    const uint32_t *hdr = plan + plan_stride - 4;
    const xyzz_t *B = hdr[1] ? ((hdr[0] & 1u) ? ping : pong) : buckets;
    if (first) {
        total[b] = B[b];
    } else {
        total[b] = E29::pack(E29::add(E29::unpack(total[b]), E29::unpack(B[b])));
    }
}

template <class C>
__device__ __forceinline__ void lds_tree_sum(xyzz_t *v, uint32_t n_pow2) {
    for (uint32_t s = n_pow2 >> 1; s >= 1; s >>= 1) {
        if (threadIdx.x < s) v[threadIdx.x] = Ec<C>::add(v[threadIdx.x], v[threadIdx.x + s]);
        __syncthreads();
    }
}

__device__ __forceinline__ xyzz_t shfl_down_point_w(const xyzz_t &p, unsigned delta, int width) {
    xyzz_t o;
    shfl_down_words<32>(reinterpret_cast<const uint32_t *>(&p), reinterpret_cast<uint32_t *>(&o), delta, width);
    return o;
}

template <class C>
__global__ void SRS_KERNEL_BOUNDS(128, 1)
    k_rowcol(const xyzz_t *__restrict__ buckets, const xyzz_t *__restrict__ ping, size_t ping_stride,
             const xyzz_t *__restrict__ pong, size_t pong_stride, const uint32_t *__restrict__ plan, size_t plan_stride,
             xyzz_t *__restrict__ rc , const Link *__restrict__ link, int from_buckets) {
    constexpr uint32_t SER = 8;
    __shared__ xyzz_t half[1];
    const uint32_t m = blockIdx.y, wave = threadIdx.x >> 6, lane = threadIdx.x & 63u;
    const uint32_t q = lane & 3u, vl = lane >> 2;
    const uint32_t *hdr = plan + (size_t)m * plan_stride + plan_stride - 4;
    const size_t ping_off = link ? (size_t)link->base[0][m] : (size_t)m * ping_stride;
    const size_t pong_off = link ? (size_t)link->base[1][m] : (size_t)m * pong_stride;
    const xyzz_t *B = (hdr[1] && !from_buckets) ? ((hdr[0] & 1u) ? ping + ping_off : pong + pong_off) : buckets + (size_t)m * NBUCKET;
    using E29 = Ec29<C>;
    xyzz_t *out = rc + (size_t)m * (RED_ROWS + RED_COLS);
    const bool is_row = blockIdx.x < RED_ROWS / 2;
    xyzz29_t acc;
    if (is_row) {
        const uint32_t hi = blockIdx.x * 2 + wave;
        const xyzz_t *src = B + (size_t)hi * RED_COLS + vl * SER;
        acc = E29::unpack(src[0]);
        xyzz_t nx = src[1];
        for (uint32_t j = 1; j < SER; ++j) {
            xyzz_t cur = nx;
            if (j + 1 < SER) nx = src[j + 1];
            acc = E29::add_quad(acc, E29::unpack(cur), q);
        }
    } else {
        const uint32_t lo = blockIdx.x - RED_ROWS / 2, sub = wave * 16 + vl;
        const xyzz_t *src = B + (size_t)(sub * SER) * RED_COLS + lo;
        acc = E29::unpack(src[0]);
        xyzz_t nx = src[RED_COLS];
        for (uint32_t j = 1; j < SER; ++j) {
            xyzz_t cur = nx;
            if (j + 1 < SER) nx = src[(size_t)(j + 1) * RED_COLS];
            acc = E29::add_quad(acc, E29::unpack(cur), q);
        }
    }
    for (unsigned d = 8; d >= 1; d >>= 1) {
        xyzz29_t o = shfl_down_point29(acc, 4 * d, 64);
        if (vl < d) acc = E29::add_quad(acc, o, q);
    }
    if (is_row) {
        if (lane == 0) out[blockIdx.x * 2 + wave] = E29::pack(acc);
        return;
    }
    if (wave == 1 && lane == 0) half[0] = E29::pack(acc);
    __syncthreads();
    if (wave == 0 && vl == 0) {
        acc = E29::add_quad(acc, E29::unpack(half[0]), q);
        if (q == 0) out[RED_ROWS + (blockIdx.x - RED_ROWS / 2)] = E29::pack(acc);
    }
}

template <class C>
__global__ void SRS_KERNEL_BOUNDS(RED_THREADS, 1)
    k_reduce_final(const xyzz_t *__restrict__ rc, xyzz_t *__restrict__ out) {
    constexpr uint32_t N = RED_COLS;
    using E29 = Ec29<C>;
    __shared__ xyzz29_t v[N];
    const uint32_t m = blockIdx.y, t = threadIdx.x >> 2, q = threadIdx.x & 3u, which = blockIdx.x;
    const xyzz_t *rows = rc + (size_t)m * (RED_ROWS + RED_COLS), *cols = rows + RED_ROWS;
    xyzz29_t x;
    if (which == 0) x = E29::add_quad(E29::unpack(rows[2 * t]), E29::unpack(rows[2 * t + 1]), q);
    else if (which == 1 || which == 3) x = E29::unpack(cols[t]);
    else x = E29::unpack(rows[2 * t + 1]);
    if (which < 2) {
        if (q == 0) v[t] = x;
        __syncthreads();
        for (uint32_t s = 1; s < N; s <<= 1) {
            const bool has = t + s < N;
            xyzz29_t o = has ? v[t + s] : E29::identity();
            __syncthreads();
            if (has) x = E29::add_quad(x, o, q);
            if (q == 0) v[t] = x;
            __syncthreads();
        }
        if (which == 0 && t == 0) x = E29::identity();
    }
    if (q == 0) v[t] = x;
    __syncthreads();
    for (uint32_t s = N >> 1; s >= 1; s >>= 1) {
        if (t < s) {
            x = E29::add_quad(x, v[t + s], q);
            if (q == 0) v[t] = x;
        }
        __syncthreads();
    }
    if (threadIdx.x == 0) out[(size_t)m * gridDim.x + which] = E29::pack(v[0]);
}

template <class C>
__global__ void SRS_KERNEL_BOUNDS(256, 1)
    k_wide_combine(const xyzz_t *__restrict__ in , xyzz_t *__restrict__ out ) {
    using E29 = Ec29<C>;
    const uint32_t which = threadIdx.x >> 6, lane = threadIdx.x & 63u, q = lane & 3u, vl = lane >> 2;
    xyzz29_t x = E29::unpack(in[vl * 4 + which]);
    if (which == 3) {
        for (uint32_t s = 1; s < NSEG_W; s <<= 1) {
            xyzz29_t o = shfl_down_point29(x, 4 * s, 64);
            if (vl + s < NSEG_W) x = E29::add_quad(x, o, q);
        }
        if (vl == 0) x = E29::identity();
    }
    for (unsigned d = NSEG_W / 2; d >= 1; d >>= 1) {
        xyzz29_t o = shfl_down_point29(x, 4 * d, 64);
        if (vl < d) x = E29::add_quad(x, o, q);
    }
    if (lane == 0) out[which] = E29::pack(x);
}

static inline uint32_t ceil_div(uint64_t a, uint64_t b) { return (uint32_t)((a + b - 1) / b); }

template <class C>
static void expand_windows(affine_t *table, uint32_t n, int nwin, int nbits, xyzz_t *tmp, hipStream_t stream) {
    for (int w = 1; w < nwin; ++w) {
        const affine_t *prev = table + (size_t)(w - 1) * n;
        affine_t *cur = table + (size_t)w * n;
        SRS_LAUNCH((k_table_step<C>), (ceil_div(n, 256)), (256), 0, stream, prev, tmp, n, nbits);
        SRS_LAUNCH((k_normalize<C>), (ceil_div(ceil_div(n, NORM_G), 128)), (128), 0, stream, (const xyzz_t *)tmp, cur, n);
    }
}

static bool wants_wide_table(size_t len) {
    static const int env_forced = [] { const char *e = std::getenv("SRS_MSM_WIDE"); return e ? std::atoi(e) : -1; }();
    const int forced = (int)tuning::get_or(tuning::MSM_WIDE, env_forced);
    if (forced == 0 || len == 0) return false;
    return forced == 1 || len >= ((size_t)1 << WIDE_MIN_KEY_LOG);
}

template <class C>
static void build_table_t(Key &k, hipStream_t stream) {
    const uint32_t n = (uint32_t)k.len;
    if (k.table_w) {
        SRS_HIP_CHECK(hipFree(k.table_w));
        k.table_w = nullptr;
    }
    if (n == 0) return;
    xyzz_t *tmp = nullptr;
    SRS_HIP_CHECK(hipMalloc((void **)&tmp, (size_t)n * sizeof(xyzz_t)));
    if (!k.compact && wants_wide_table(n) && hipMalloc((void **)&k.table_w, (size_t)n * NWIN_W * sizeof(affine_t)) != hipSuccess) {
        (void)hipGetLastError();
        k.table_w = nullptr;
    }
    if (k.table_w) {
        SRS_HIP_CHECK(hipMemcpyAsync(k.table_w, k.table, (size_t)n * sizeof(affine_t), hipMemcpyDeviceToDevice, stream));
        expand_windows<C>(k.table_w, n, NWIN_W, WBITS_W, tmp, stream);
        const size_t total_w = (size_t)n * NWIN_W;
        SRS_LAUNCH((k_table_form<C>), (ceil_div(total_w, 256)), (256), 0, stream, k.table_w, total_w);
    }
    const int nwin = k.compact ? NWIN_COMPACT : NWIN;
    expand_windows<C>(k.table, n, nwin, WBITS, tmp, stream);
    const size_t total = (size_t)n * nwin;
    SRS_LAUNCH((k_table_form<C>), (ceil_div(total, 256)), (256), 0, stream, k.table, total);
    SRS_HIP_CHECK(hipStreamSynchronize(stream));
    SRS_HIP_CHECK(hipFree(tmp));
}

template <class C>
static void generate_t(Key &k, uint64_t seed, hipStream_t stream) {
    const uint32_t n = (uint32_t)k.len;
    if (n == 0) return;
    xyzz_t *tmp = nullptr;
    SRS_HIP_CHECK(hipMalloc((void **)&tmp, (size_t)n * sizeof(xyzz_t)));
    SRS_LAUNCH((k_gen_bases<C>), (ceil_div(n, 128)), (128), 0, stream, tmp, n, seed, k.rank, k.world);
    SRS_LAUNCH((k_normalize<C>), (ceil_div(ceil_div(n, NORM_G), 128)), (128), 0, stream, (const xyzz_t *)tmp, k.table, n);
    SRS_HIP_CHECK(hipStreamSynchronize(stream));
    SRS_HIP_CHECK(hipFree(tmp));
}
void generate_bases(Key &k, uint64_t seed, hipStream_t stream) {
    if (k.curve == 0) generate_t<Bn256>(k, seed, stream); else generate_t<Grumpkin>(k, seed, stream);
}

size_t count_off_curve(const Key &k, hipStream_t stream) {
    if (k.len == 0) return 0;
    uint32_t *d_bad = nullptr, bad = 0;
    SRS_HIP_CHECK(hipMalloc((void **)&d_bad, sizeof(uint32_t)));
    SRS_HIP_CHECK(hipMemsetAsync(d_bad, 0, sizeof(uint32_t), stream));
    const uint32_t n = (uint32_t)k.len;
    if (k.curve == 0) SRS_LAUNCH((k_on_curve<Bn256>), (ceil_div(n, 256)), (256), 0, stream, (const affine_t *)k.table, n, d_bad);
    else SRS_LAUNCH((k_on_curve<Grumpkin>), (ceil_div(n, 256)), (256), 0, stream, (const affine_t *)k.table, n, d_bad);
    SRS_HIP_CHECK(hipMemcpyAsync(&bad, d_bad, sizeof(uint32_t), hipMemcpyDeviceToHost, stream));
    SRS_HIP_CHECK(hipStreamSynchronize(stream));
    (void)hipFree(d_bad);
    return bad;
}

void read_bases(const Key &k, affine_t *out_dev, hipStream_t stream) {
    if (k.len == 0) return;
    if (k.curve == 0) SRS_LAUNCH((k_table_unform<Bn256>), (ceil_div(k.len, 256)), (256), 0, stream, (const affine_t *)k.table, out_dev, k.len);
    else SRS_LAUNCH((k_table_unform<Grumpkin>), (ceil_div(k.len, 256)), (256), 0, stream, (const affine_t *)k.table, out_dev, k.len);
}

void build_table(Key &k, hipStream_t stream) {
    if (k.curve == 0) build_table_t<Bn256>(k, stream); else build_table_t<Grumpkin>(k, stream);
}

int choose_windows(Key &k) {
    k.compact = tuning::get_or(tuning::MSM_COMPACT, 0) == 1;
    if (k.compact && (uint64_t)NWIN_COMPACT * k.len > PAY_ENDO) {
        set_error("compact key (msm_compact = 1): 8 x " + std::to_string(k.len) + " table entries do not fit below the endomorphism flag (2^30)");
        throw DeviceError{4};
    }
    return k.compact ? NWIN_COMPACT : NWIN;
}
size_t table_bytes(const Key &k) {
    if (!k.table) return 0;
    return k.len * sizeof(affine_t) * ((k.compact ? NWIN_COMPACT : NWIN) + (k.table_w ? NWIN_W : 0));
}


static uint32_t l0_log_for(uint64_t M) {
    const int forced = (int)tuning::get_or(tuning::MSM_L0, 0);
    if (forced >= 1 && forced <= 7) return (uint32_t)forced;
    if (M < (1ull << 20)) return 2;
    if (M < (1ull << 22)) return 3;
    uint32_t lg = ACC_L0_LOG;
    while (lg < 7 && (M >> (lg + 1)) >= (5ull << 20)) ++lg;
    return lg;
}

static uint32_t acc1_quad_max() {
    const int64_t lg = tuning::get_or(tuning::MSM_QUAD_MAX, 0);
    return (lg >= 1 && lg <= 24) ? (1u << lg) : ACC1_QUAD_MAX;
}

static int levels_for(uint64_t parts) {
    int levels = 1;
    while (parts > FINAL_FANIN && levels < MAX_LEVELS) {
        parts = (parts + ACC_L1 - 1) / ACC_L1;
        ++levels;
    }
    return levels;
}

static bool use_two_pass(uint64_t M, uint32_t batch) {
    const int forced = (int)tuning::get_or(tuning::MSM_SORT, 0);
    if (forced == 1) return false;
    if (forced == 2) return true;
    return M * batch >= TWO_PASS_MIN_SLOTS;
}

static uint32_t slot_log() {
    const int64_t lg = tuning::get_or(tuning::MSM_SLOT_LOG, 0);
    return (lg >= 2 && lg <= 8) ? (uint32_t)lg : SLOT_LOG;
}
static uint32_t slot_want_cap() { return 4u; }

struct LevelShape {
    uint64_t M;
    int levels;
    size_t plan_stride;
    uint64_t cap0, cap1;
    uint32_t quad_max;
};
struct SetShape : LevelShape {
    bool two_pass;
    uint32_t tile, tiles;
};
struct NarrowShape : SetShape { uint32_t l0_log; };
struct SlotShape : SetShape { uint32_t S, nred; };
struct WideShape : LevelShape { uint32_t l0_log, T, tiles_g; };

static void sort_shape(SetShape &h, uint32_t n_max, uint32_t batch) {
    h.M = (uint64_t)n_max * NWIN;
    h.quad_max = acc1_quad_max();
    h.two_pass = use_two_pass(h.M, batch);
    h.tile = (uint32_t)((h.M * batch + SORT_TARGET_BLOCKS - 1) / SORT_TARGET_BLOCKS);
    h.tile = (h.tile + 1023u) & ~1023u;
    if (h.tile < SORT_TILE_MIN) h.tile = SORT_TILE_MIN;
    h.tiles = ceil_div(n_max, h.tile);
}
static NarrowShape narrow_shape(uint32_t n_max, uint32_t batch) {
    NarrowShape h;
    sort_shape(h, n_max, batch);
    h.l0_log = l0_log_for(h.M);
    h.levels = levels_for((h.M + (1ull << h.l0_log) - 1) >> h.l0_log);
    h.plan_stride = (size_t)(h.levels + 1) * (NBUCKET + 1) + 4;
    h.cap0 = (h.M >> h.l0_log) + NBUCKET + 1;
    h.cap1 = h.cap0 / ACC_L1 + NBUCKET + 1;
    return h;
}
static SlotShape slot_shape(uint32_t n_max, uint32_t batch) {
    SlotShape h;
    sort_shape(h, n_max, batch);
    const uint32_t lg = slot_log();
    h.S = 1u << lg;
    h.nred = (lg + 2) / 3;
    h.cap0 = std::min<uint64_t>((uint64_t)NBUCKET * h.S, (h.M >> SLOT_L0_MIN_LOG) + NBUCKET);
    h.cap1 = h.cap0 / ACC_L1 + NBUCKET + 1;
    h.levels = levels_for(h.cap0);
    h.plan_stride = (size_t)(h.levels + 2) * (NBUCKET + 1) + 4;
    return h;
}
static WideShape wide_shape(uint32_t n) {
    WideShape w;
    w.M = (uint64_t)n * NWIN_W;
    w.quad_max = acc1_quad_max();
    w.l0_log = l0_log_for(w.M);
    w.levels = levels_for((w.M + (1ull << w.l0_log) - 1) >> w.l0_log);
    w.plan_stride = (size_t)(w.levels + 1) * (NBUCKET + 1) + 4;
    w.cap0 = (w.M >> w.l0_log) + (uint64_t)NSEG_W * (NBUCKET + 1);
    w.cap1 = w.cap0 / ACC_L1 + (uint64_t)NSEG_W * (NBUCKET + 1);
    w.T = ceil_div(n, WIDE_TILE);
    w.tiles_g = SORT_TARGET_BLOCKS;
    return w;
}

struct Sizer {
    size_t used = 0;
    template <class T>
    T *take(size_t count) {
        used += Arena::pad(count * sizeof(T));
        return nullptr;
    }
};
template <class Walk>
static size_t sized(Walk walk) {
    Sizer s;
    walk(s);
    return s.used;
}
template <class Walk>
static auto carve(Arena &A, Walk walk) {
    const size_t need = sized(walk);
    A.reserve(need);
    A.reset();
    const auto bufs = walk(A);
    if (A.used != need) {
        set_error("internal: msm workspace: the arena walk and the sizer disagree");
        throw DeviceError{5};
    }
    return bufs;
}

struct SetBufs {
    xyzz_t *d_out, *ping, *pong, *rc;
    uint16_t *dig, *tb;
    uint32_t *sorted, *count, *cursor, *plan;
    uint16_t *gkey;
    uint32_t *gpay, *tile_hist;
};
struct NarrowBufs : SetBufs { xyzz_t *buckets; };
struct SlotBufs : SetBufs { xyzz_t *red_a, *red_b; };
template <class W>
static void take_set_head(W &A, const SetShape &h, uint32_t batch, SetBufs &b) {
    b.d_out = A.template take<xyzz_t>(3 * (size_t)batch);
    b.dig = A.template take<uint16_t>(h.M * batch);
    b.sorted = A.template take<uint32_t>(h.M * batch);
    b.count = A.template take<uint32_t>((size_t)NBUCKET * batch);
    b.cursor = A.template take<uint32_t>((size_t)NBUCKET * batch);
    b.plan = A.template take<uint32_t>(h.plan_stride * batch);
    b.ping = A.template take<xyzz_t>(h.cap0 * batch);
    b.tb = A.template take<uint16_t>(h.cap0 * batch);
    b.pong = A.template take<xyzz_t>(h.cap1 * batch);
}
template <class W>
static void take_set_tail(W &A, const SetShape &h, uint32_t batch, SetBufs &b) {
    b.rc = A.template take<xyzz_t>((size_t)(RED_ROWS + RED_COLS) * batch);
    b.gkey = h.two_pass ? A.template take<uint16_t>(h.M * batch) : nullptr;
    b.gpay = h.two_pass ? A.template take<uint32_t>(h.M * batch) : nullptr;
    b.tile_hist = h.two_pass ? A.template take<uint32_t>((size_t)SEG * (SORT_TARGET_BLOCKS + 2 * NWIN) * batch) : nullptr;
}
template <class W>
static NarrowBufs narrow_layout(W &A, const NarrowShape &h, uint32_t batch) {
    NarrowBufs b;
    take_set_head(A, h, batch, b);
    b.buckets = A.template take<xyzz_t>((size_t)NBUCKET * batch);
    take_set_tail(A, h, batch, b);
    return b;
}
template <class W>
static SlotBufs slot_layout(W &A, const SlotShape &h, uint32_t batch) {
    SlotBufs b;
    take_set_head(A, h, batch, b);
    b.red_a = A.template take<xyzz_t>((size_t)NBUCKET * (h.S / 8 + 1) * batch);
    b.red_b = A.template take<xyzz_t>((size_t)NBUCKET * (h.S / 64 + 1) * batch);
    take_set_tail(A, h, batch, b);
    return b;
}
struct WideBufs {
    xyzz_t *d_out, *d_seg, *ping, *pong, *buckets, *rc;
    uint16_t *gkey, *gkey2, *tb;
    uint32_t *gpay, *gpay2, *tile_cnt, *tile_hist;
    uint32_t *seg3;
    uint32_t *sorted, *count, *cursor, *plan;
    Link *link;
};
template <class W>
static WideBufs wide_layout(W &A, const WideShape &w) {
    WideBufs b;
    b.d_out = A.template take<xyzz_t>(4);
    b.d_seg = A.template take<xyzz_t>(4 * NSEG_W);
    b.gkey = A.template take<uint16_t>(w.M);
    b.gpay = A.template take<uint32_t>(w.M);
    b.sorted = A.template take<uint32_t>(w.M);
    b.tile_cnt = A.template take<uint32_t>((size_t)NSEG_W * w.T);
    b.gkey2 = A.template take<uint16_t>(w.M);
    b.gpay2 = A.template take<uint32_t>(w.M);
    b.tile_hist = A.template take<uint32_t>((size_t)SEG * w.tiles_g);
    b.seg3 = A.template take<uint32_t>(4 * (NSEG_W + 2));
    b.link = A.template take<Link>(1);
    b.count = A.template take<uint32_t>((size_t)NSEG_W * NBUCKET);
    b.cursor = A.template take<uint32_t>((size_t)NSEG_W * NBUCKET);
    b.plan = A.template take<uint32_t>(w.plan_stride * NSEG_W);
    b.ping = A.template take<xyzz_t>(w.cap0);
    b.tb = A.template take<uint16_t>(w.cap0);
    b.pong = A.template take<xyzz_t>(w.cap1);
    b.buckets = A.template take<xyzz_t>((size_t)NSEG_W * NBUCKET);
    b.rc = A.template take<xyzz_t>((size_t)NSEG_W * (RED_ROWS + RED_COLS));
    return b;
}

size_t workspace_bytes(uint32_t n_max, uint32_t batch) {
    return sized([&](auto &A) { return narrow_layout(A, narrow_shape(n_max, batch), batch); });
}
static size_t workspace_bytes_slots(uint32_t n_max, uint32_t batch) {
    return sized([&](auto &A) { return slot_layout(A, slot_shape(n_max, batch), batch); });
}
static size_t workspace_bytes_wide(uint32_t n) {
    return sized([&](auto &A) { return wide_layout(A, wide_shape(n)); });
}

template <class C, class LaunchPlan>
static void sort_front(const Key &k, const SetShape &h, const SetBufs &b, const fe_t *const *scalars_dev, const uint32_t *n_host,
                       const uint32_t *base_host, uint32_t batch, uint32_t n_max, int is_mont, hipStream_t stream, LaunchPlan launch_plan,
                       bool group_maps, uint32_t arr) {
    BatchDesc bd;
    for (uint32_t m = 0; m < BATCH_ARGS; ++m) {
        bd.ptr[m] = m < batch ? scalars_dev[m] : nullptr;
        bd.n[m] = m < batch ? n_host[m] : 0;
        bd.base[m] = (m < batch && base_host) ? base_host[m] : 0;
    }
    const uint32_t s_rank = k.compact_scalars ? 0u : k.rank, s_world = k.compact_scalars ? 1u : k.world;
    const size_t M = (size_t)h.M;
    const auto digits = k.compact ? &k_digits<C, true> : &k_digits<C, false>;
    const auto group = k.compact ? &k_group<true> : &k_group<false>;
    const auto scatter = k.compact ? &k_scatter<true> : &k_scatter<false>;
    SRS_LAUNCH(digits, (ceil_div(n_max, 256), batch), (256), 0, stream, bd, b.dig, M, is_mont, s_rank, s_world, b.count,
               (uint32_t)(NBUCKET * batch));
    SRS_LAUNCH(k_hist, (h.tiles, NWIN, batch), (SORT_THREADS), 0, stream, (const uint16_t *)b.dig, M, bd, b.count, h.tile, b.tile_hist);
    launch_plan();
    if (h.two_pass) {
        const uint32_t T1 = h.tiles * NWIN;
        SRS_LAUNCH(k_scan_seg, (SEG, batch), (1024), 0, stream, b.tile_hist, T1, (const uint32_t *)b.plan, h.plan_stride);
        SRS_LAUNCH(group, (h.tiles, NWIN, batch), (SORT_THREADS), 0, stream, (const uint16_t *)b.dig, M, bd, (const uint32_t *)b.tile_hist,
                   b.gkey, b.gpay, M, (uint32_t)k.len, h.tile, group_maps ? (const uint32_t *)b.plan : nullptr,
                   group_maps ? h.plan_stride : (size_t)0, group_maps ? b.tb : nullptr, group_maps ? (size_t)h.cap0 : (size_t)0,
                   group_maps ? arr : 0u);
        SRS_LAUNCH(k_scatter2, (8 * ceil_div(ceil_div(M, SORT_TILE2), 8), batch), (SORT_THREADS), 0, stream, (const uint16_t *)b.gkey,
                   (const uint32_t *)b.gpay, M, (const uint32_t *)b.plan, h.plan_stride, b.cursor, b.sorted, M, (uint32_t)SORT_TILE2);
    } else {
        SRS_LAUNCH(scatter, (h.tiles, NWIN, batch), (SORT_THREADS), 0, stream, (const uint16_t *)b.dig, M, bd, b.cursor, b.sorted, M,
                   (uint32_t)k.len, h.tile);
    }
    if (!(h.two_pass && group_maps))
        SRS_LAUNCH(k_expand, (NBUCKET / 4, batch), (256), 0, stream, (const uint32_t *)b.plan, h.plan_stride, b.tb, (size_t)h.cap0,
                   (const Link *)nullptr, arr);
}

struct Parts {
    const uint32_t *plan; size_t plan_stride;
    xyzz_t *ping; size_t stride0;
    xyzz_t *pong; size_t stride1;
    const Link *link;
};

template <class C>
static void accum_levels(const Parts &p, const LevelShape &h, uint64_t cap_inc, uint32_t batch, hipStream_t stream) {
    xyzz_t *cur = p.ping, *nxt = p.pong;
    size_t cur_stride = p.stride0, nxt_stride = p.stride1;
    uint64_t cap = h.cap0;
    for (int level = 1; level < h.levels; ++level) {
        cap = cap / ACC_L1 + cap_inc;
        SRS_LAUNCH((k_accum1<C>), (ceil_div(std::max<uint64_t>(cap, 4 * std::min<uint64_t>(cap, h.quad_max)), ACC_THREADS), batch),
                   (ACC_THREADS), 0, stream, (const xyzz_t *)cur, cur_stride, p.plan, h.plan_stride, level, nxt, nxt_stride, (uint32_t)ACC_L1,
                   p.link, h.quad_max);
        std::swap(cur, nxt);
        std::swap(cur_stride, nxt_stride);
    }
}

template <class C>
static void reduce_buckets(const Parts &p, uint32_t nmsm, const xyzz_t *from, int from_buckets, xyzz_t *rc, uint32_t sums, xyzz_t *d_sums,
                           hipStream_t stream) {
    SRS_LAUNCH((k_rowcol<C>), (RED_ROWS / 2 + RED_COLS, nmsm), (128), 0, stream, from, (const xyzz_t *)p.ping, p.stride0,
               (const xyzz_t *)p.pong, p.stride1, p.plan, p.plan_stride, rc, p.link, from_buckets);
    SRS_LAUNCH((k_reduce_final<C>), (sums, nmsm), (RED_THREADS), 0, stream, (const xyzz_t *)rc, d_sums);
}

static void land(Key &k, const xyzz_t *d_out, size_t n, uint32_t slot, hipStream_t stream) {
    if (!k.h_result) SRS_HIP_CHECK(hipHostMalloc(&k.h_result, 3 * (size_t)BATCH_ARGS * LANDING_SLOTS * sizeof(xyzz_t)));
    xyzz_t *dst = static_cast<xyzz_t *>(k.h_result) + 3 * (size_t)BATCH_ARGS * slot;
    SRS_HIP_CHECK(hipMemcpyAsync(dst, d_out, n * sizeof(xyzz_t), hipMemcpyDeviceToHost, stream));
}

template <class C>
static bool enqueue_t(Key &k, const fe_t *const *scalars_dev, const uint32_t *n_host, const uint32_t *base_host, uint32_t batch,
                      uint32_t n_max, int is_mont, hipStream_t stream, uint32_t slot, Fold fold) {
    if (n_max == 0) return false;
    const NarrowShape h = narrow_shape(n_max, batch);
    const NarrowBufs b = carve(k.arena, [&](auto &A) { return narrow_layout(A, h, batch); });
    sort_front<C>(k, h, b, scalars_dev, n_host, base_host, batch, n_max, is_mont, stream, [&] {
        SRS_LAUNCH(k_plan, (batch, h.levels + 1), (PLAN_THREADS), 0, stream, (const uint32_t *)b.count, b.cursor, b.plan, h.plan_stride,
                   h.levels, h.l0_log, (uint32_t)ACC_L1_LOG, (const uint32_t *)nullptr);
    }, false, 1u);
    const Parts p{b.plan, h.plan_stride, b.ping, (size_t)h.cap0, b.pong, (size_t)h.cap1, nullptr};
    const uint64_t units = std::accumulate(n_host, n_host + batch, (uint64_t)0);
    const auto accum0 = k.compact ? &k_accum0c<C> : &k_accum0<C>;
    SRS_LAUNCH_TIMED("msm_accum0", units, accum0, (ceil_div(h.cap0, ACC_THREADS), batch), (ACC_THREADS), 0, stream,
                     (const uint32_t *)b.sorted, (size_t)h.M, p.plan, p.plan_stride, (const uint16_t *)b.tb, p.stride0,
                     (const affine_t *)k.table, p.ping, p.stride0, 1u << h.l0_log, p.link);
    accum_levels<C>(p, h, NBUCKET + 1, batch, stream);
    SRS_LAUNCH((k_accum_final<C>), (NBUCKET / (FINAL_THREADS / 64), batch), (FINAL_THREADS), 0, stream, (const xyzz_t *)p.ping, p.stride0,
               (const xyzz_t *)p.pong, p.stride1, p.plan, p.plan_stride, b.buckets, p.link);
    const xyzz_t *red_from = b.buckets;
    int from_buckets = 0;
    if (fold != FOLD_NONE) {
        if (!k.fold_buckets) SRS_HIP_CHECK(hipMalloc((void **)&k.fold_buckets, (size_t)NBUCKET * sizeof(xyzz_t)));
        SRS_LAUNCH((k_bucket_fold<C>), (NBUCKET / 64), (64), 0, stream, (const xyzz_t *)b.buckets, (const xyzz_t *)p.ping,
                   (const xyzz_t *)p.pong, p.plan, p.plan_stride, k.fold_buckets, fold == FOLD_FIRST ? 1 : 0);
        if (fold != FOLD_LAST) return true;
        red_from = k.fold_buckets;
        from_buckets = 1;
    }
    reduce_buckets<C>(p, batch, red_from, from_buckets, b.rc, 3, b.d_out, stream);
    land(k, b.d_out, 3 * (size_t)batch, slot, stream);
    k.landing[slot].wide = false;
    return true;
}

static bool use_wide(const Key &k, uint32_t n_max, uint32_t batch);
static bool use_slots(const Key &k, uint32_t n_max, uint32_t batch, Fold fold) {
    const int mode = (int)tuning::get_or(tuning::MSM_SLOTS, 1);
    if (mode == 0) return false;
    if (fold != FOLD_NONE) return batch == 1;
    return mode == 2 && !use_wide(k, n_max, batch);
}

template <class C>
static bool enqueue_slots_t(Key &k, const fe_t *const *scalars_dev, const uint32_t *n_host, const uint32_t *base_host, uint32_t batch,
                            uint32_t n_max, int is_mont, hipStream_t stream, uint32_t slot, Fold fold) {
    if (n_max == 0) return false;
    const bool first = fold == FOLD_NONE || fold == FOLD_FIRST, last = fold == FOLD_NONE || fold == FOLD_LAST;
    const SlotShape h = slot_shape(n_max, batch);
    const uint32_t S = h.S;
    if (first) {
        k.slot_s = S;
        k.seq = 0;
        k.commit_ovf = k.expect_ovf;
        const size_t need = (size_t)batch * NBUCKET * S;
        if (k.slots_pts < need) {
            if (k.slots) SRS_HIP_CHECK(hipFree(k.slots));
            k.slots = nullptr;
            k.slots_pts = 0;
            SRS_HIP_CHECK(hipMalloc((void **)&k.slots, need * sizeof(xyzz_t)));
            k.slots_pts = need;
        }
        if (!k.used) SRS_HIP_CHECK(hipMalloc((void **)&k.used, 2 * (size_t)BATCH_ARGS * NBUCKET));
        if (!k.h_ovf) {
            SRS_HIP_CHECK(hipHostMalloc((void **)&k.h_ovf, 2 * (size_t)LANDING_SLOTS * BATCH_ARGS * sizeof(uint32_t)));
            for (size_t i = 0; i < 2 * (size_t)LANDING_SLOTS * BATCH_ARGS; ++i) k.h_ovf[i] = 0;
        }
    } else if (k.slot_s != S || batch != 1) {
        set_error("internal: msm slot mode: a commit's sets must share the slot layout");
        throw DeviceError{5};
    }
    const uint8_t *used_prev = k.used + (size_t)(k.seq & 1u) * BATCH_ARGS * NBUCKET;
    uint8_t *used_next = k.used + (size_t)((k.seq + 1) & 1u) * BATCH_ARGS * NBUCKET;
    ++k.seq;

    const SlotBufs b = carve(k.arena, [&](auto &A) { return slot_layout(A, h, batch); });
    const uint32_t arr = (uint32_t)h.levels + 1;
    sort_front<C>(k, h, b, scalars_dev, n_host, base_host, batch, n_max, is_mont, stream, [&] {
        SRS_LAUNCH(k_plan_s, (batch, h.levels + 2), (PLAN_THREADS), 0, stream, (const uint32_t *)b.count, b.cursor, b.plan, h.plan_stride,
                   h.levels, S, (uint32_t)ACC_L1_LOG, used_prev, used_next, first ? 1 : 0, k.h_ovf + (size_t)slot * BATCH_ARGS, slot_want_cap());
    }, true, arr);
    const Parts p{b.plan, h.plan_stride, b.ping, (size_t)h.cap0, b.pong, (size_t)h.cap1, nullptr};
    const uint64_t units = std::accumulate(n_host, n_host + batch, (uint64_t)0);
    const auto accum0s = k.compact ? &k_accum0sc<C> : &k_accum0s<C>;
    SRS_LAUNCH_TIMED("msm_accum0", units, accum0s, (ceil_div(h.cap0, ACC_THREADS), batch), (ACC_THREADS), 0, stream,
                     (const uint32_t *)b.sorted, (size_t)h.M, p.plan, p.plan_stride, arr, (const uint16_t *)b.tb, p.stride0,
                     (const affine_t *)k.table, k.slots, S, used_prev, first ? 1 : 0, p.ping, p.stride0);
    if (k.commit_ovf) {
        accum_levels<C>(p, h, NBUCKET + 1, batch, stream);
        SRS_LAUNCH((k_ovf_final<C>), (NBUCKET / (FINAL_THREADS / 64), batch), (FINAL_THREADS), 0, stream, (const xyzz_t *)p.ping, p.stride0,
                   (const xyzz_t *)p.pong, p.stride1, p.plan, p.plan_stride, k.slots, S, first ? 1 : 0);
    }
    k.landing[slot] = {false, true, k.commit_ovf, batch};
    ++k.stat_slot_sets;
    if (!last) return true;
    const xyzz_t *in = k.slots;
    uint32_t in_pb = S;
    xyzz_t *outs[2] = {b.red_a, b.red_b};
    for (uint32_t l = 0; l < h.nred; ++l) {
        const uint32_t out_pb = (in_pb + 7) / 8, n_out = NBUCKET * out_pb;
        xyzz_t *out = outs[l & 1u];
        const uint8_t *used = l == 0 ? used_next : nullptr;
        const int extra = (l == 0 && k.commit_ovf) ? (int)S - 1 : -1;
        if (l + 1 == h.nred) {
            SRS_LAUNCH((k_slot_reduce<C, true>), (ceil_div((uint64_t)n_out * 4, 256), batch), (256), 0, stream, in, in_pb, used, (size_t)NBUCKET, extra,
                       out, out_pb);
        } else {
            SRS_LAUNCH((k_slot_reduce<C, false>), (ceil_div(n_out, 256), batch), (256), 0, stream, in, in_pb, used, (size_t)NBUCKET, extra, out,
                       out_pb);
        }
        in = out;
        in_pb = out_pb;
    }
    reduce_buckets<C>(p, batch, in, 1, b.rc, 3, b.d_out, stream);
    land(k, b.d_out, 3 * (size_t)batch, slot, stream);
    return true;
}

bool overflow_missed(const Key &k, uint32_t slot) {
    if (slot >= LANDING_SLOTS || !k.landing[slot].slot_mode || k.landing[slot].ovf_on || !k.h_ovf) return false;
    for (uint32_t m = 0; m < k.landing[slot].batch; ++m)
        if (k.h_ovf[(size_t)slot * BATCH_ARGS + m]) return true;
    return false;
}
void note_commit(Key &k, const uint32_t *slots_used, uint32_t n_slots, uint64_t scalars) {
    bool any = false, slot_sets = false;
    uint64_t entries = 0;
    for (uint32_t i = 0; i < n_slots; ++i) {
        const uint32_t sl = slots_used[i];
        if (sl >= LANDING_SLOTS || !k.landing[sl].slot_mode || !k.h_ovf) continue;
        slot_sets = true;
        for (uint32_t m = 0; m < k.landing[sl].batch; ++m) entries += k.h_ovf[(size_t)(LANDING_SLOTS + sl) * BATCH_ARGS + m];
        bool hot = false;
        for (uint32_t m = 0; m < k.landing[sl].batch; ++m) hot = hot || k.h_ovf[(size_t)sl * BATCH_ARGS + m] != 0;
        if (hot) ++k.stat_hot_sets;
        any = any || hot;
    }
    constexpr uint32_t COLD_COMMITS = 3;
    if (!slot_sets) {
        k.last_entries = k.last_scalars = 0;
        return;
    }
    k.last_entries = entries;
    k.last_scalars = scalars;
    if (any) {
        k.expect_ovf = true;
        k.cold_streak = 0;
    } else if (k.expect_ovf && ++k.cold_streak >= COLD_COMMITS) {
        k.expect_ovf = false;
        k.cold_streak = 0;
    }
}

static bool use_wide(const Key &k, uint32_t n_max, uint32_t batch) {
    const int min_log = (int)tuning::get_or(tuning::MSM_WIDE_MIN, (int64_t)WIDE_MIN_N_LOG);
    return k.table_w != nullptr && batch == 1 && n_max >= (1u << min_log);
}

template <class C>
static bool enqueue_wide_t(Key &k, const fe_t *scalars_dev, uint32_t n, uint32_t base, int is_mont, hipStream_t stream, uint32_t slot) {
    const WideShape w = wide_shape(n);
    const WideBufs b = carve(k.arena, [&](auto &A) { return wide_layout(A, w); });
    uint32_t *seg_total = b.seg3, *seg_off = b.seg3 + (NSEG_W + 2), *tile_base = b.seg3 + 2 * (NSEG_W + 2), *tile_base2 = b.seg3 + 3 * (NSEG_W + 2);

    WideDesc wd;
    wd.ptr = scalars_dev;
    wd.n = n;
    wd.base = base;
    wd.rank = k.compact_scalars ? 0u : k.rank;
    wd.world = k.compact_scalars ? 1u : k.world;
    wd.is_mont = is_mont;
    const uint32_t table_stride = (uint32_t)k.len;

    SRS_HIP_CHECK(hipMemsetAsync(seg_total, 0, (NSEG_W + 1) * sizeof(uint32_t), stream));
    SRS_HIP_CHECK(hipMemsetAsync(b.count, 0, (size_t)NSEG_W * NBUCKET * sizeof(uint32_t), stream));
    SRS_LAUNCH((k_seg_pass<C, false>), (w.T), (WIDE_THREADS), 0, stream, wd, b.tile_cnt, w.T, seg_total, (uint16_t *)nullptr,
               (uint32_t *)nullptr, table_stride);
    const uint32_t small_tiles = (w.M >> 19) < 64 ? 1u : 0u, tile2_host = small_tiles ? SORT_TILE2 / 4 : SORT_TILE2;
    SRS_LAUNCH(k_seg_scan, (NSEG_W), (1024), 0, stream, b.tile_cnt, w.T, (const uint32_t *)seg_total, seg_off, tile_base, tile_base2, small_tiles);
    SRS_LAUNCH((k_seg_pass<C, true>), (w.T), (WIDE_THREADS), 0, stream, wd, b.tile_cnt, w.T, seg_total, b.gkey, b.gpay, table_stride);
    SRS_LAUNCH(k_hist_g, (w.tiles_g), (SORT_THREADS), 0, stream, (const uint16_t *)b.gkey, (const uint32_t *)seg_off,
               (const uint32_t *)tile_base, b.count, b.tile_hist);
    SRS_LAUNCH(k_plan, (NSEG_W, w.levels + 1), (PLAN_THREADS), 0, stream, (const uint32_t *)b.count, b.cursor, b.plan, w.plan_stride, w.levels,
               w.l0_log, (uint32_t)ACC_L1_LOG, (const uint32_t *)seg_off);
    SRS_LAUNCH(k_scan_seg_g, (SEG, NSEG_W), (1024), 0, stream, b.tile_hist, w.tiles_g, (const uint32_t *)tile_base, (const uint32_t *)b.plan,
               w.plan_stride);
    SRS_LAUNCH(k_group_g, (w.tiles_g), (SORT_THREADS), 0, stream, (const uint16_t *)b.gkey, (const uint32_t *)b.gpay, (const uint32_t *)seg_off,
               (const uint32_t *)tile_base, (const uint32_t *)b.tile_hist, b.gkey2, b.gpay2);
    SRS_LAUNCH(k_scatter2_g, (8 * ceil_div(ceil_div(w.M, tile2_host) + NSEG_W, 8)), (SORT_THREADS), 0, stream, (const uint16_t *)b.gkey2,
               (const uint32_t *)b.gpay2, (const uint32_t *)seg_off, (const uint32_t *)tile_base2, b.cursor, b.sorted);
    SRS_LAUNCH(k_link, (1), (64), 0, stream, (const uint32_t *)b.plan, w.plan_stride, w.levels, b.link);
    const Parts p{b.plan, w.plan_stride, b.ping, 0, b.pong, 0, b.link};
    SRS_LAUNCH(k_expand, (NBUCKET / 4, NSEG_W), (256), 0, stream, p.plan, p.plan_stride, b.tb, (size_t)0, p.link, 1u);
    SRS_LAUNCH_TIMED("msm_accum0", n, (k_accum0<C>), (ceil_div(w.cap0, ACC_THREADS)), (ACC_THREADS), 0, stream, (const uint32_t *)b.sorted,
                     (size_t)0, p.plan, p.plan_stride, (const uint16_t *)b.tb, (size_t)0, (const affine_t *)k.table_w, p.ping, (size_t)0,
                     1u << w.l0_log, p.link);
    accum_levels<C>(p, w, (uint64_t)NSEG_W * (NBUCKET + 1), 1, stream);
    SRS_LAUNCH((k_accum_final<C>), (NBUCKET / (FINAL_THREADS / 64), NSEG_W), (FINAL_THREADS), 0, stream, (const xyzz_t *)p.ping, p.stride0,
               (const xyzz_t *)p.pong, p.stride1, p.plan, p.plan_stride, b.buckets, p.link);
    reduce_buckets<C>(p, NSEG_W, b.buckets, 0, b.rc, 4, b.d_seg, stream);
    SRS_LAUNCH((k_wide_combine<C>), (1), (256), 0, stream, (const xyzz_t *)b.d_seg, b.d_out);
    land(k, b.d_out, 4, slot, stream);
    k.landing[slot].wide = true;
    return true;
}

template <class C>
static void finish_t(Key &k, uint32_t batch, uint32_t slot, bool launched, xyzz_t *result_host) {
    if (!launched) {
        for (uint32_t m = 0; m < batch; ++m) result_host[m] = Ec<C>::identity();
        return;
    }
    const xyzz_t *raw = static_cast<const xyzz_t *>(k.h_result) + 3 * (size_t)BATCH_ARGS * slot;
    using F = typename C::F;
    fe_t c = F::one();
    for (int d = 0; d < 5; ++d) c = F::halve(c);
    std::vector<xyzz_t> two(3 * (size_t)batch + (k.landing[slot].wide ? 1 : 0));
    for (size_t i = 0; i < two.size(); ++i) {
        two[i].x = F::mul(raw[i].x, c);
        two[i].y = F::mul(raw[i].y, c);
        two[i].zz = F::mul(raw[i].zz, c);
        two[i].zzz = F::mul(raw[i].zzz, c);
    }
    for (uint32_t m = 0; m < batch; ++m) {
        xyzz_t a = Ec<C>::add(Ec<C>::dbl(two[3 * m]), two[3 * m + 2]);
        for (uint32_t j = 1; j < RED_COLS; j <<= 1) a = Ec<C>::dbl(a);
        result_host[m] = Ec<C>::add(a, two[3 * m + 1]);
    }
    if (k.landing[slot].wide) {
        xyzz_t u = two[3];
        for (uint32_t j = 1; j < NBUCKET; j <<= 1) u = Ec<C>::dbl(u);
        result_host[0] = Ec<C>::add(result_host[0], u);
    }
}

bool enqueue(Key &k, const fe_t *const *scalars_dev, const uint32_t *n_host, const uint32_t *base_host, uint32_t batch, int is_mont,
             hipStream_t stream, uint32_t slot, Fold fold) {
    if (batch > BATCH_ARGS || slot >= LANDING_SLOTS) {
        set_error("internal: msm::enqueue batch / slot out of range");
        throw DeviceError{5};
    }
    if (fold != FOLD_NONE && batch != 1) {
        set_error("internal: msm::enqueue fold needs one MSM per set");
        throw DeviceError{5};
    }
    if (batch == 1 && fold == FOLD_NONE && use_wide(k, n_host[0], 1)) {
        const uint32_t base = base_host ? base_host[0] : 0;
        k.landing[slot].slot_mode = false;
        ++k.stat_other_sets;
        return k.curve == 0 ? enqueue_wide_t<Bn256>(k, scalars_dev[0], n_host[0], base, is_mont, stream, slot)
                            : enqueue_wide_t<Grumpkin>(k, scalars_dev[0], n_host[0], base, is_mont, stream, slot);
    }
    uint32_t n_max = 0;
    for (uint32_t m = 0; m < batch; ++m) n_max = std::max(n_max, n_host[m]);
    const bool first = fold == FOLD_NONE || fold == FOLD_FIRST;
    const bool slots = first ? use_slots(k, n_max, batch, fold) : k.slot_s != 0;
    if (slots)
        return k.curve == 0 ? enqueue_slots_t<Bn256>(k, scalars_dev, n_host, base_host, batch, n_max, is_mont, stream, slot, fold)
                            : enqueue_slots_t<Grumpkin>(k, scalars_dev, n_host, base_host, batch, n_max, is_mont, stream, slot, fold);
    if (first) k.slot_s = 0;
    k.landing[slot].slot_mode = false;
    ++k.stat_other_sets;
    return k.curve == 0 ? enqueue_t<Bn256>(k, scalars_dev, n_host, base_host, batch, n_max, is_mont, stream, slot, fold)
                        : enqueue_t<Grumpkin>(k, scalars_dev, n_host, base_host, batch, n_max, is_mont, stream, slot, fold);
}
void finish(Key &k, uint32_t batch, uint32_t slot, bool launched, xyzz_t *result_host) {
    if (k.curve == 0) finish_t<Bn256>(k, batch, slot, launched, result_host); else finish_t<Grumpkin>(k, batch, slot, launched, result_host);
}
void reserve(Key &k, uint32_t n_max, uint32_t batch) {
    size_t b = use_wide(k, n_max, batch) ? std::max(workspace_bytes_wide(n_max), workspace_bytes(n_max, batch)) : workspace_bytes(n_max, batch);
    if (batch == 1) b = std::max(b, workspace_bytes_slots(n_max, batch));
    k.arena.reserve(b);
}

void release(Key &k) {
    if (k.table_w) (void)hipFree(k.table_w);
    k.table_w = nullptr;
    if (k.fold_buckets) (void)hipFree(k.fold_buckets);
    k.fold_buckets = nullptr;
    if (k.h_result) (void)hipHostFree(k.h_result);
    k.h_result = nullptr;
    if (k.slots) (void)hipFree(k.slots);
    k.slots = nullptr;
    k.slots_pts = 0;
    if (k.used) (void)hipFree(k.used);
    k.used = nullptr;
    if (k.h_ovf) (void)hipHostFree(k.h_ovf);
    k.h_ovf = nullptr;
    k.arena.release();
}

void run(Key &k, const fe_t *const *scalars_dev, const uint32_t *n_host, uint32_t batch, int is_mont,
         hipStream_t stream, xyzz_t *result_host) {
    for (uint32_t at = 0; at < batch;) {
        uint32_t b = std::min<uint32_t>(BATCH_ARGS, batch - at);
        if (use_wide(k, n_host[at], 1)) b = 1;
        bool launched = enqueue(k, scalars_dev + at, n_host + at, nullptr, b, is_mont, stream, 0);
        if (launched) {
            SRS_HIP_CHECK(hipStreamSynchronize(stream));
            SRS_HIP_CHECK(hipGetLastError());
            const uint32_t sl = 0;
            if (overflow_missed(k, sl)) {
                k.expect_ovf = true;
                ++k.stat_redo;
                launched = enqueue(k, scalars_dev + at, n_host + at, nullptr, b, is_mont, stream, 0);
                SRS_HIP_CHECK(hipStreamSynchronize(stream));
                SRS_HIP_CHECK(hipGetLastError());
            }
            uint64_t total = 0;
            for (uint32_t m = 0; m < b; ++m) total += n_host[at + m];
            note_commit(k, &sl, 1, total);
        }
        finish(k, b, 0, launched, result_host + at);
        prof::collect();
        at += b;
    }
}

}
}
```

sirius_amd/csrc/tuning.h:

```cpp
#pragma once
#include <cstdint>

namespace srs {
namespace tuning {

enum Id : int {
    MSM_SORT = 0,
    MSM_L0,
    MSM_WIDE,
    MSM_WIDE_MIN,
    MSM_SLOTS,
    MSM_SLOT_LOG,
    MSM_EXPECT_OVF,
    MSM_QUAD_MAX,
    COMMIT_CHUNKS,
    PG_F_EVAL,
    PG_G_FFT,
    JIT_ALWAYS,
    NO_JIT,
    MSM_COMPACT,
    PG_COMPAT_TREE,
    N_TUNABLES
};

constexpr int64_t UNSET = INT64_MIN;

int64_t get(Id id);
inline int64_t get_or(Id id, int64_t dflt) {
    const int64_t v = get(id);
    return v == UNSET ? dflt : v;
}
int set(const char *name, int64_t value);
int64_t get_by_name(const char *name, int *found);
void reset();
const char *name_of(int id);

}
}
```

sirius_amd/csrc/tuning.hip:

```cpp
#include "tuning.h"

#include <atomic>
#include <cstring>

namespace srs {
namespace tuning {

static std::atomic<int64_t> g_val[N_TUNABLES];
static const char *const kNames[N_TUNABLES] = {"msm_sort", "msm_l0", "msm_wide", "msm_wide_min", "msm_slots", "msm_slot_log", "msm_expect_ovf",
                                               "msm_quad_max", "commit_chunks", "pg_f_eval", "pg_g_fft", "jit_always", "no_jit", "msm_compact", "pg_compat_tree"};
static struct Init {
    Init() { for (auto &v : g_val) v.store(UNSET, std::memory_order_relaxed); }
} g_init;

int64_t get(Id id) { return g_val[id].load(std::memory_order_relaxed); }
const char *name_of(int id) { return id >= 0 && id < N_TUNABLES ? kNames[id] : nullptr; }
static int find(const char *name) {
    if (!name) return -1;
    for (int i = 0; i < N_TUNABLES; ++i)
        if (std::strcmp(kNames[i], name) == 0) return i;
    return -1;
}
int set(const char *name, int64_t value) {
    const int i = find(name);
    if (i < 0) return -1;
    g_val[i].store(value, std::memory_order_relaxed);
    return 0;
}
int64_t get_by_name(const char *name, int *found) {
    const int i = find(name);
    if (found) *found = i >= 0;
    return i < 0 ? UNSET : get((Id)i);
}
void reset() { for (auto &v : g_val) v.store(UNSET, std::memory_order_relaxed); }

}
}
```

Before: 99.29.

## Precompute per-part descriptors and store slot buckets in native 29-bit form

Replaces the per-thread bucket map (uint16 bucket id plus plan lookups) with a precomputed 16-byte part descriptor holding start, end, slot index and resume/overflow flags, so the slot accumulate kernel does one vector load instead of several dependent plan reads. Slot buckets now stay in the 29-bit limb xyzz29 layout and are loaded and stored as 9 uint4 words, avoiding a pack/unpack on every resume and reduce. It also adds an optional non-power-of-two part length knob. The trade-off is a larger descriptor buffer (tb sized by tb_words), bigger slot storage at 144 bytes per point, and extra descriptor-writing work in the grouping or expand kernel.

```diff
diff --git a/sirius_amd/csrc/msm.h b/sirius_amd/csrc/msm.h
--- a/sirius_amd/csrc/msm.h
+++ b/sirius_amd/csrc/msm.h
@@ -8,6 +8,7 @@
 #include <cstdlib>
 
 namespace srs {
+struct xyzz29_t;
 namespace msm {
 
 constexpr int WBITS = 16;
@@ -67,7 +68,7 @@
     void *h_result = nullptr;
     struct Landing { bool wide = false, slot_mode = false, ovf_on = false; uint32_t batch = 0; } landing[LANDING_SLOTS];
     xyzz_t *fold_buckets = nullptr;
-    xyzz_t *slots = nullptr;
+    xyzz29_t *slots = nullptr;
     size_t slots_pts = 0;
     uint8_t *used = nullptr;
     uint32_t *h_ovf = nullptr;
diff --git a/sirius_amd/csrc/msm.hip b/sirius_amd/csrc/msm.hip
--- a/sirius_amd/csrc/msm.hip
+++ b/sirius_amd/csrc/msm.hip
@@ -19,6 +19,30 @@
         if (tp[mid] <= t) lo = mid; else hi = mid;
     }
     return lo;
+}
+
+struct PartDesc {
+    uint32_t s, e, slot, flags;
+};
+static_assert(sizeof(PartDesc) == 16, "PartDesc travels as one 16-byte word");
+constexpr uint32_t PART_RESUME = 1u, PART_OVF = 2u;
+
+__device__ __forceinline__ void write_part_descs(const uint32_t *__restrict__ pl, size_t plan_stride, uint32_t arr, uint32_t S,
+                                                 const uint8_t *__restrict__ used, PartDesc *__restrict__ out, uint32_t b, uint32_t lane) {
+    const uint32_t *tp = pl + (size_t)arr * (NBUCKET + 1);
+    const uint32_t t0 = tp[b], parts = tp[b + 1] - t0;
+    if (parts == 0) return;
+    const uint32_t o0 = pl[b], o1 = pl[b + 1], ov = pl[(NBUCKET + 1) + b], len = pl[plan_stride - 2];
+    const uint32_t was = used ? (uint32_t)used[b] : 0u;
+    for (uint32_t p = lane; p < parts; p += 64) {
+        PartDesc d;
+        d.s = o0 + p * len;
+        d.e = d.s + len < o1 ? d.s + len : o1;
+        const bool regular = p < S - 1;
+        d.slot = regular ? b * S + p : ov + (p - (S - 1));
+        d.flags = regular ? (p < was ? PART_RESUME : 0u) : PART_OVF;
+        out[t0 + p] = d;
+    }
 }
 
 template <class C>
@@ -280,20 +304,18 @@
 __global__ void SRS_KERNEL_BOUNDS(SORT_THREADS, 1)
     k_group(const uint16_t *__restrict__ dig, size_t dig_stride, BatchDesc bd, const uint32_t *__restrict__ tile_hist,
             uint16_t *__restrict__ gkey, uint32_t *__restrict__ gpay, size_t g_stride, uint32_t table_stride, uint32_t SORT_TILE,
-            const uint32_t *__restrict__ plan, size_t plan_stride, uint16_t *__restrict__ tb, size_t tb_stride, uint32_t arr) {
+            const uint32_t *__restrict__ plan, size_t plan_stride, PartDesc *__restrict__ desc, size_t desc_stride, uint32_t arr, uint32_t S,
+            const uint8_t *__restrict__ used_prev) {
     __shared__ uint32_t cur[SEG], cnt[SEG], lb[SEG], sc[64];
     __shared__ uint32_t spay[GRP_SUB];
     __shared__ uint16_t skey[GRP_SUB];
     const uint32_t m = blockIdx.z, w = blockIdx.y, tid = threadIdx.x;
-    if (tb) {
-        const uint32_t *tp = plan + (size_t)m * plan_stride + (size_t)arr * (NBUCKET + 1);
-        uint16_t *map = tb + (size_t)m * tb_stride;
+    if (desc) {
         const uint32_t waves = gridDim.x * gridDim.y * (blockDim.x >> 6);
         const uint32_t wv = (blockIdx.y * gridDim.x + blockIdx.x) * (blockDim.x >> 6) + (tid >> 6), lane = tid & 63u;
-        for (uint32_t b = wv; b < NBUCKET; b += waves) {
-            const uint32_t s = tp[b], e = tp[b + 1];
-            for (uint32_t t = s + lane; t < e; t += 64) map[t] = (uint16_t)b;
-        }
+        for (uint32_t b = wv; b < NBUCKET; b += waves)
+            write_part_descs(plan + (size_t)m * plan_stride, plan_stride, arr, S, used_prev ? used_prev + (size_t)m * NBUCKET : nullptr,
+                             desc + (size_t)m * desc_stride, b, lane);
     }
     const uint32_t n = bd.n[m];
     const uint32_t lo = blockIdx.x * SORT_TILE;
@@ -917,22 +939,27 @@
     }
 }
 
-__device__ __forceinline__ uint32_t slot_l0_log(uint32_t total_entries, uint32_t S, uint32_t want_cap) {
+__device__ __forceinline__ uint32_t slot_part_len(uint32_t total_entries, uint32_t S, uint32_t want_cap, uint32_t force_len) {
     const uint32_t mean = total_entries / NBUCKET;
     uint32_t r = 0;
     while ((r + 1) * (r + 1) <= mean) ++r;
     const uint32_t thresh = mean + 6 * r + 1;
+    if (force_len) {
+        const uint32_t fit = (thresh + S - 2) / (S - 1), top = 1u << SLOT_L0_MAX_LOG;
+        const uint32_t len = force_len > fit ? force_len : fit;
+        return len < top ? len : top;
+    }
     uint32_t lg = SLOT_L0_MIN_LOG;
     while (((thresh + (1u << lg) - 1) >> lg) > S - 1 && lg < SLOT_L0_MAX_LOG) ++lg;
     uint32_t want = 0;
     while (want < want_cap && (total_entries >> (19 + want + 1)) != 0) ++want;
-    return lg > want ? lg : want;
+    return 1u << (lg > want ? lg : want);
 }
 
 __global__ void SRS_KERNEL_BOUNDS(PLAN_THREADS, 1)
     k_plan_s(const uint32_t *__restrict__ count, uint32_t *__restrict__ cursor, uint32_t *__restrict__ plan, size_t plan_stride, int nlevels,
              uint32_t S, uint32_t l1_log, const uint8_t *__restrict__ used_prev, uint8_t *__restrict__ used_next, int first,
-             uint32_t *__restrict__ h_ovf, uint32_t want_cap) {
+             uint32_t *__restrict__ h_ovf, uint32_t want_cap, uint32_t force_len) {
     constexpr uint32_t PER = NBUCKET / PLAN_THREADS;
     __shared__ uint32_t tile[NBUCKET + NBUCKET / PER];
     __shared__ uint32_t lds[64];
@@ -956,13 +983,24 @@
     for (uint32_t j = 0; j < PER; ++j) local += tile[base + j];
     uint32_t total_entries;
     uint32_t run = block_exclusive_scan(local, lds, &total_entries);
-    const uint32_t l0_log = slot_l0_log(total_entries, S, want_cap);
+    const uint32_t l0 = slot_part_len(total_entries, S, want_cap, force_len);
+    const bool l0_pow2 = (l0 & (l0 - 1)) == 0;
+    uint32_t l0_sh = 0;
+    while ((1u << (l0_sh + 1)) <= l0) ++l0_sh;
+    const uint32_t l0_rcp = (uint32_t)(0x100000000ull / l0);
+    auto parts_of = [&](uint32_t c) -> uint32_t {
+        const uint32_t x = c + l0 - 1;
+        if (l0_pow2) return x >> l0_sh;
+        uint32_t q = __umulhi(x, l0_rcp);
+        if (x - q * l0 >= l0) ++q;
+        return q;
+    };
     uint32_t total = total_entries;
     const bool dense = role == (uint32_t)nlevels + 1;
     const uint32_t lv = role >= 2 && !dense ? role - 1 : 0;
     auto value = [&](uint32_t c) -> uint32_t {
         if (role == 0) return c;
-        uint32_t p = (c + (1u << l0_log) - 1) >> l0_log;
+        uint32_t p = parts_of(c);
         if (dense) return p;
         p = p > S - 1 ? p - (S - 1) : 0u;
         for (uint32_t l = 0; l < lv; ++l) p = (p + (1u << l1_log) - 1) >> l1_log;
@@ -976,7 +1014,7 @@
             const uint32_t c = tile[base + j];
             local += value(c);
             if (!dense) {
-                const uint32_t p = (c + (1u << l0_log) - 1) >> l0_log, o = p > S - 1 ? p - (S - 1) : 0u;
+                const uint32_t p = parts_of(c), o = p > S - 1 ? p - (S - 1) : 0u;
                 mx = o > mx ? o : mx;
             }
         }
@@ -990,7 +1028,7 @@
             if (role == 1 && t == 0) {
                 pl[plan_stride - 4] = (uint32_t)needed;
                 pl[plan_stride - 3] = 0;
-                pl[plan_stride - 2] = l0_log;
+                pl[plan_stride - 2] = l0;
             }
             if ((int)role - 1 >= needed) return;
         }
@@ -1069,6 +1107,37 @@
     for (uint32_t t = s + lane; t < e; t += 64) out[t] = (uint16_t)b;
 }
 
+__global__ void SRS_KERNEL_BOUNDS(256, 1)
+    k_expand_s(const uint32_t *__restrict__ plan, size_t plan_stride, PartDesc *__restrict__ desc, size_t desc_stride, uint32_t arr, uint32_t S,
+               const uint8_t *__restrict__ used_prev) {
+    const uint32_t m = blockIdx.y;
+    write_part_descs(plan + (size_t)m * plan_stride, plan_stride, arr, S, used_prev ? used_prev + (size_t)m * NBUCKET : nullptr,
+                     desc + (size_t)m * desc_stride, blockIdx.x * 4 + (threadIdx.x >> 6), threadIdx.x & 63u);
+}
+
+static_assert(sizeof(xyzz29_t) == 144, "a slot is 9 x 16 bytes");
+__device__ __forceinline__ xyzz29_t slot_load(const xyzz29_t *__restrict__ p) {
+    xyzz29_t o;
+    const uint4 *src = reinterpret_cast<const uint4 *>(p);
+    uint32_t *w = reinterpret_cast<uint32_t *>(&o);
+#pragma unroll
+    for (int i = 0; i < 9; ++i) {
+        const uint4 v = src[i];
+        w[4 * i] = v.x; w[4 * i + 1] = v.y; w[4 * i + 2] = v.z; w[4 * i + 3] = v.w;
+    }
+    return o;
+}
+__device__ __forceinline__ void slot_store(xyzz29_t *__restrict__ p, const xyzz29_t &a) {
+    uint4 *dst = reinterpret_cast<uint4 *>(p);
+    const uint32_t *w = reinterpret_cast<const uint32_t *>(&a);
+#pragma unroll
+    for (int i = 0; i < 9; ++i) {
+        uint4 v;
+        v.x = w[4 * i]; v.y = w[4 * i + 1]; v.z = w[4 * i + 2]; v.w = w[4 * i + 3];
+        dst[i] = v;
+    }
+}
+
 template <class C, bool COMPACT>
 __device__ __forceinline__ aff29_t load_entry(const affine_t &p, uint32_t v) {
     aff29_t q = Ec29<C>::load_raw(p);
@@ -1087,7 +1156,7 @@
 
 template <class C, bool COMPACT>
 __device__ __forceinline__ xyzz29_t accumulate_part(const uint32_t *__restrict__ src, uint32_t s, uint32_t e, const affine_t *__restrict__ table,
-                                                    const xyzz_t *__restrict__ init) {
+                                                    const xyzz29_t *__restrict__ init) {
     using E29 = Ec29<C>;
     using F = typename E29::F;
     bool exc = false;
@@ -1098,7 +1167,7 @@
         affine_t p = table[entry_index<COMPACT>(v)];
         uint32_t j = s;
         if (init) {
-            acc = E29::unpack(*init);
+            acc = slot_load(init);
         } else {
             affine_t pn = p;
             uint32_t vnn = 0;
@@ -1131,7 +1200,7 @@
         }
     }
     if (exc) {
-        acc = init ? E29::unpack(*init) : E29::identity();
+        acc = init ? slot_load(init) : E29::identity();
 #pragma unroll 1
         for (uint32_t j = s; j < e; ++j) {
             const uint32_t v = src[j];
@@ -1279,47 +1348,40 @@
 
 template <class C, bool COMPACT>
 __device__ __forceinline__ void accum0s_thread(const uint32_t *__restrict__ sorted, size_t sorted_stride, const uint32_t *__restrict__ plan,
-                                               size_t plan_stride, uint32_t arr, const uint16_t *__restrict__ tb, size_t tb_stride,
-                                               const affine_t *__restrict__ table, xyzz_t *__restrict__ slots, uint32_t S,
-                                               const uint8_t *__restrict__ used_prev, int first, xyzz_t *__restrict__ ovf, size_t ovf_stride) {
+                                               size_t plan_stride, uint32_t arr, const PartDesc *__restrict__ desc, size_t desc_stride,
+                                               const affine_t *__restrict__ table, xyzz29_t *__restrict__ slots, uint32_t S,
+                                               xyzz_t *__restrict__ ovf, size_t ovf_stride) {
     const uint32_t m = blockIdx.y;
     const uint32_t t = blockIdx.x * blockDim.x + threadIdx.x;
-    const uint32_t *off = plan + (size_t)m * plan_stride;
-    const uint32_t *tp = off + (size_t)arr * (NBUCKET + 1);
-    if (t >= tp[NBUCKET]) return;
-    const uint32_t *tpo = off + (NBUCKET + 1);
-    const uint32_t l0 = 1u << off[plan_stride - 2];
-    const uint32_t b = tb[(size_t)m * tb_stride + t];
-    const uint32_t part = t - tp[b];
-    uint32_t s = off[b] + part * l0;
-    uint32_t e = off[b + 1];
-    if (e > s + l0) e = s + l0;
+    if (t >= plan[(size_t)m * plan_stride + (size_t)arr * (NBUCKET + 1) + NBUCKET]) return;
+    const uint4 dw = *reinterpret_cast<const uint4 *>(desc + (size_t)m * desc_stride + t);
+    const uint32_t s = dw.x, e = dw.y, at = dw.z, flags = dw.w;
     const uint32_t *src = sorted + (size_t)m * sorted_stride;
     using E29 = Ec29<C>;
-    const bool regular = part < S - 1;
-    xyzz_t *slot = regular ? slots + ((size_t)m * NBUCKET + b) * S + part : ovf + (size_t)m * ovf_stride + tpo[b] + (part - (S - 1));
-    const bool resume = regular && !first && part < (uint32_t)used_prev[(size_t)m * NBUCKET + b];
-    *slot = E29::pack(accumulate_part<C, COMPACT>(src, s, e, table, resume ? slot : nullptr));
+    xyzz29_t *slot = slots + (size_t)m * NBUCKET * S + ((flags & PART_OVF) ? 0u : at);
+    const xyzz29_t acc = accumulate_part<C, COMPACT>(src, s, e, table, (flags & PART_RESUME) ? slot : nullptr);
+    if (flags & PART_OVF) ovf[(size_t)m * ovf_stride + at] = E29::pack(acc);
+    else slot_store(slot, acc);
 }
 template <class C>
 __global__ void SRS_KERNEL_BOUNDS(ACC_THREADS, 1)
     k_accum0s(const uint32_t *__restrict__ sorted, size_t sorted_stride, const uint32_t *__restrict__ plan, size_t plan_stride, uint32_t arr,
-              const uint16_t *__restrict__ tb, size_t tb_stride, const affine_t *__restrict__ table, xyzz_t *__restrict__ slots, uint32_t S,
-              const uint8_t *__restrict__ used_prev, int first, xyzz_t *__restrict__ ovf, size_t ovf_stride) {
-    accum0s_thread<C, false>(sorted, sorted_stride, plan, plan_stride, arr, tb, tb_stride, table, slots, S, used_prev, first, ovf, ovf_stride);
+              const PartDesc *__restrict__ desc, size_t desc_stride, const affine_t *__restrict__ table, xyzz29_t *__restrict__ slots, uint32_t S,
+              xyzz_t *__restrict__ ovf, size_t ovf_stride) {
+    accum0s_thread<C, false>(sorted, sorted_stride, plan, plan_stride, arr, desc, desc_stride, table, slots, S, ovf, ovf_stride);
 }
 template <class C>
 __global__ void SRS_KERNEL_BOUNDS(ACC_THREADS, 1)
     k_accum0sc(const uint32_t *__restrict__ sorted, size_t sorted_stride, const uint32_t *__restrict__ plan, size_t plan_stride, uint32_t arr,
-               const uint16_t *__restrict__ tb, size_t tb_stride, const affine_t *__restrict__ table, xyzz_t *__restrict__ slots, uint32_t S,
-               const uint8_t *__restrict__ used_prev, int first, xyzz_t *__restrict__ ovf, size_t ovf_stride) {
-    accum0s_thread<C, true>(sorted, sorted_stride, plan, plan_stride, arr, tb, tb_stride, table, slots, S, used_prev, first, ovf, ovf_stride);
+               const PartDesc *__restrict__ desc, size_t desc_stride, const affine_t *__restrict__ table, xyzz29_t *__restrict__ slots, uint32_t S,
+               xyzz_t *__restrict__ ovf, size_t ovf_stride) {
+    accum0s_thread<C, true>(sorted, sorted_stride, plan, plan_stride, arr, desc, desc_stride, table, slots, S, ovf, ovf_stride);
 }
 
 template <class C>
 __global__ void SRS_KERNEL_BOUNDS(FINAL_THREADS, 1)
     k_ovf_final(const xyzz_t *__restrict__ ping, size_t ping_stride, const xyzz_t *__restrict__ pong, size_t pong_stride,
-                const uint32_t *__restrict__ plan, size_t plan_stride, xyzz_t *__restrict__ slots, uint32_t S, int first) {
+                const uint32_t *__restrict__ plan, size_t plan_stride, xyzz29_t *__restrict__ slots, uint32_t S, int first) {
     const uint32_t m = blockIdx.y;
     const uint32_t level = plan[(size_t)m * plan_stride + plan_stride - 4];
     const xyzz_t *in = (level & 1u) ? ping + (size_t)m * ping_stride : pong + (size_t)m * pong_stride;
@@ -1327,10 +1389,10 @@
     const uint32_t lane = threadIdx.x & 63u;
     const uint32_t b = blockIdx.x * (blockDim.x >> 6) + (threadIdx.x >> 6);
     const uint32_t s = tp[b], e = tp[b + 1];
-    xyzz_t *dst = slots + ((size_t)m * NBUCKET + b) * S + (S - 1);
+    xyzz29_t *dst = slots + ((size_t)m * NBUCKET + b) * S + (S - 1);
     using E29 = Ec29<C>;
     if (e == s) {
-        if (first && lane == 0) *dst = E29::pack(E29::identity());
+        if (first && lane == 0) slot_store(dst, E29::identity());
         return;
     }
     xyzz29_t acc = E29::identity();
@@ -1340,14 +1402,19 @@
         if (lane < d) acc = E29::add(acc, other);
     }
     if (lane == 0) {
-        if (!first) acc = E29::add(acc, E29::unpack(*dst));
-        *dst = E29::pack(acc);
-    }
-}
-
-template <class C, bool QUAD>
+        if (!first) acc = E29::add(acc, slot_load(dst));
+        acc.y = E29::F::normalize(acc.y);
+        slot_store(dst, acc);
+    }
+}
+
+template <class C>
+__device__ __forceinline__ xyzz29_t reduce_input(const xyzz_t *__restrict__ p) { return Ec29<C>::unpack(*p); }
+template <class C>
+__device__ __forceinline__ xyzz29_t reduce_input(const xyzz29_t *__restrict__ p) { return slot_load(p); }
+template <class C, bool QUAD, class In>
 __global__ void SRS_KERNEL_BOUNDS(256, 1)
-    k_slot_reduce(const xyzz_t *__restrict__ in, uint32_t in_pb, const uint8_t *__restrict__ used, size_t used_stride, int extra,
+    k_slot_reduce(const In *__restrict__ in, uint32_t in_pb, const uint8_t *__restrict__ used, size_t used_stride, int extra,
                   xyzz_t *__restrict__ out, uint32_t out_pb) {
     using E29 = Ec29<C>;
     const uint32_t m = blockIdx.y;
@@ -1355,11 +1422,11 @@
     if (t >= NBUCKET * out_pb) return;
     const uint32_t g = t / NBUCKET, b = t % NBUCKET;
     const uint32_t lim = used ? (uint32_t)used[(size_t)m * used_stride + b] : in_pb;
-    const xyzz_t *src = in + ((size_t)m * NBUCKET + b) * in_pb;
+    const In *src = in + ((size_t)m * NBUCKET + b) * in_pb;
     xyzz29_t acc = E29::identity();
     for (uint32_t idx = g; idx < in_pb; idx += out_pb) {
         if (!(idx < lim || (int)idx == extra)) continue;
-        const xyzz29_t x = E29::unpack(src[idx]);
+        const xyzz29_t x = reduce_input<C>(src + idx);
         if (QUAD) acc = E29::add_quad(acc, x, q); else acc = E29::add(acc, x);
     }
     if (!QUAD || q == 0) out[((size_t)m * NBUCKET + b) * out_pb + g] = E29::pack(acc);
@@ -1641,6 +1708,10 @@
     return (lg >= 2 && lg <= 8) ? (uint32_t)lg : SLOT_LOG;
 }
 static uint32_t slot_want_cap() { return 4u; }
+static uint32_t slot_force_len() {
+    const int64_t len = tuning::get_or(tuning::MSM_SLOT_LEN, 0);
+    return (len >= (int64_t)(1u << SLOT_L0_MIN_LOG) && len <= 64) ? (uint32_t)len : 0u;
+}
 
 struct LevelShape {
     uint64_t M;
@@ -1651,6 +1722,7 @@
 };
 struct SetShape : LevelShape {
     bool two_pass;
+    uint32_t tb_words;
     uint32_t tile, tiles;
 };
 struct NarrowShape : SetShape { uint32_t l0_log; };
@@ -1669,6 +1741,7 @@
 static NarrowShape narrow_shape(uint32_t n_max, uint32_t batch) {
     NarrowShape h;
     sort_shape(h, n_max, batch);
+    h.tb_words = 1;
     h.l0_log = l0_log_for(h.M);
     h.levels = levels_for((h.M + (1ull << h.l0_log) - 1) >> h.l0_log);
     h.plan_stride = (size_t)(h.levels + 1) * (NBUCKET + 1) + 4;
@@ -1680,6 +1753,7 @@
     SlotShape h;
     sort_shape(h, n_max, batch);
     const uint32_t lg = slot_log();
+    h.tb_words = sizeof(PartDesc) / sizeof(uint16_t);
     h.S = 1u << lg;
     h.nred = (lg + 2) / 3;
     h.cap0 = std::min<uint64_t>((uint64_t)NBUCKET * h.S, (h.M >> SLOT_L0_MIN_LOG) + NBUCKET);
@@ -1747,7 +1821,7 @@
     b.cursor = A.template take<uint32_t>((size_t)NBUCKET * batch);
     b.plan = A.template take<uint32_t>(h.plan_stride * batch);
     b.ping = A.template take<xyzz_t>(h.cap0 * batch);
-    b.tb = A.template take<uint16_t>(h.cap0 * batch);
+    b.tb = A.template take<uint16_t>(h.cap0 * batch * h.tb_words);
     b.pong = A.template take<xyzz_t>(h.cap1 * batch);
 }
 template <class W>
@@ -1817,10 +1891,14 @@
     return sized([&](auto &A) { return wide_layout(A, wide_shape(n)); });
 }
 
+struct SlotMaps {
+    uint32_t S;
+    const uint8_t *used_prev;
+};
 template <class C, class LaunchPlan>
 static void sort_front(const Key &k, const SetShape &h, const SetBufs &b, const fe_t *const *scalars_dev, const uint32_t *n_host,
                        const uint32_t *base_host, uint32_t batch, uint32_t n_max, int is_mont, hipStream_t stream, LaunchPlan launch_plan,
-                       bool group_maps, uint32_t arr) {
+                       const SlotMaps *sm, uint32_t arr) {
     BatchDesc bd;
     for (uint32_t m = 0; m < BATCH_ARGS; ++m) {
         bd.ptr[m] = m < batch ? scalars_dev[m] : nullptr;
@@ -1840,18 +1918,20 @@
         const uint32_t T1 = h.tiles * NWIN;
         SRS_LAUNCH(k_scan_seg, (SEG, batch), (1024), 0, stream, b.tile_hist, T1, (const uint32_t *)b.plan, h.plan_stride);
         SRS_LAUNCH(group, (h.tiles, NWIN, batch), (SORT_THREADS), 0, stream, (const uint16_t *)b.dig, M, bd, (const uint32_t *)b.tile_hist,
-                   b.gkey, b.gpay, M, (uint32_t)k.len, h.tile, group_maps ? (const uint32_t *)b.plan : nullptr,
-                   group_maps ? h.plan_stride : (size_t)0, group_maps ? b.tb : nullptr, group_maps ? (size_t)h.cap0 : (size_t)0,
-                   group_maps ? arr : 0u);
+                   b.gkey, b.gpay, M, (uint32_t)k.len, h.tile, (const uint32_t *)b.plan, h.plan_stride,
+                   sm ? reinterpret_cast<PartDesc *>(b.tb) : nullptr, (size_t)h.cap0, arr, sm ? sm->S : 0u, sm ? sm->used_prev : nullptr);
         SRS_LAUNCH(k_scatter2, (8 * ceil_div(ceil_div(M, SORT_TILE2), 8), batch), (SORT_THREADS), 0, stream, (const uint16_t *)b.gkey,
                    (const uint32_t *)b.gpay, M, (const uint32_t *)b.plan, h.plan_stride, b.cursor, b.sorted, M, (uint32_t)SORT_TILE2);
     } else {
         SRS_LAUNCH(scatter, (h.tiles, NWIN, batch), (SORT_THREADS), 0, stream, (const uint16_t *)b.dig, M, bd, b.cursor, b.sorted, M,
                    (uint32_t)k.len, h.tile);
     }
-    if (!(h.two_pass && group_maps))
+    if (!sm)
         SRS_LAUNCH(k_expand, (NBUCKET / 4, batch), (256), 0, stream, (const uint32_t *)b.plan, h.plan_stride, b.tb, (size_t)h.cap0,
                    (const Link *)nullptr, arr);
+    else if (!h.two_pass)
+        SRS_LAUNCH(k_expand_s, (NBUCKET / 4, batch), (256), 0, stream, (const uint32_t *)b.plan, h.plan_stride,
+                   reinterpret_cast<PartDesc *>(b.tb), (size_t)h.cap0, arr, sm->S, sm->used_prev);
 }
 
 struct Parts {
@@ -1899,7 +1979,7 @@
     sort_front<C>(k, h, b, scalars_dev, n_host, base_host, batch, n_max, is_mont, stream, [&] {
         SRS_LAUNCH(k_plan, (batch, h.levels + 1), (PLAN_THREADS), 0, stream, (const uint32_t *)b.count, b.cursor, b.plan, h.plan_stride,
                    h.levels, h.l0_log, (uint32_t)ACC_L1_LOG, (const uint32_t *)nullptr);
-    }, false, 1u);
+    }, nullptr, 1u);
     const Parts p{b.plan, h.plan_stride, b.ping, (size_t)h.cap0, b.pong, (size_t)h.cap1, nullptr};
     const uint64_t units = std::accumulate(n_host, n_host + batch, (uint64_t)0);
     const auto accum0 = k.compact ? &k_accum0c<C> : &k_accum0<C>;
@@ -1949,7 +2029,7 @@
             if (k.slots) SRS_HIP_CHECK(hipFree(k.slots));
             k.slots = nullptr;
             k.slots_pts = 0;
-            SRS_HIP_CHECK(hipMalloc((void **)&k.slots, need * sizeof(xyzz_t)));
+            SRS_HIP_CHECK(hipMalloc((void **)&k.slots, need * sizeof(xyzz29_t)));
             k.slots_pts = need;
         }
         if (!k.used) SRS_HIP_CHECK(hipMalloc((void **)&k.used, 2 * (size_t)BATCH_ARGS * NBUCKET));
@@ -1967,16 +2047,18 @@
 
     const SlotBufs b = carve(k.arena, [&](auto &A) { return slot_layout(A, h, batch); });
     const uint32_t arr = (uint32_t)h.levels + 1;
+    const SlotMaps sm{S, first ? nullptr : used_prev};
     sort_front<C>(k, h, b, scalars_dev, n_host, base_host, batch, n_max, is_mont, stream, [&] {
         SRS_LAUNCH(k_plan_s, (batch, h.levels + 2), (PLAN_THREADS), 0, stream, (const uint32_t *)b.count, b.cursor, b.plan, h.plan_stride,
-                   h.levels, S, (uint32_t)ACC_L1_LOG, used_prev, used_next, first ? 1 : 0, k.h_ovf + (size_t)slot * BATCH_ARGS, slot_want_cap());
-    }, true, arr);
+                   h.levels, S, (uint32_t)ACC_L1_LOG, used_prev, used_next, first ? 1 : 0, k.h_ovf + (size_t)slot * BATCH_ARGS, slot_want_cap(),
+                   slot_force_len());
+    }, &sm, arr);
     const Parts p{b.plan, h.plan_stride, b.ping, (size_t)h.cap0, b.pong, (size_t)h.cap1, nullptr};
     const uint64_t units = std::accumulate(n_host, n_host + batch, (uint64_t)0);
     const auto accum0s = k.compact ? &k_accum0sc<C> : &k_accum0s<C>;
     SRS_LAUNCH_TIMED("msm_accum0", units, accum0s, (ceil_div(h.cap0, ACC_THREADS), batch), (ACC_THREADS), 0, stream,
-                     (const uint32_t *)b.sorted, (size_t)h.M, p.plan, p.plan_stride, arr, (const uint16_t *)b.tb, p.stride0,
-                     (const affine_t *)k.table, k.slots, S, used_prev, first ? 1 : 0, p.ping, p.stride0);
+                     (const uint32_t *)b.sorted, (size_t)h.M, p.plan, p.plan_stride, arr, reinterpret_cast<const PartDesc *>(b.tb), p.stride0,
+                     (const affine_t *)k.table, k.slots, S, p.ping, p.stride0);
     if (k.commit_ovf) {
         accum_levels<C>(p, h, NBUCKET + 1, batch, stream);
         SRS_LAUNCH((k_ovf_final<C>), (NBUCKET / (FINAL_THREADS / 64), batch), (FINAL_THREADS), 0, stream, (const xyzz_t *)p.ping, p.stride0,
@@ -1985,20 +2067,22 @@
     k.landing[slot] = {false, true, k.commit_ovf, batch};
     ++k.stat_slot_sets;
     if (!last) return true;
-    const xyzz_t *in = k.slots;
+    const xyzz_t *in = nullptr;
     uint32_t in_pb = S;
     xyzz_t *outs[2] = {b.red_a, b.red_b};
     for (uint32_t l = 0; l < h.nred; ++l) {
         const uint32_t out_pb = (in_pb + 7) / 8, n_out = NBUCKET * out_pb;
         xyzz_t *out = outs[l & 1u];
-        const uint8_t *used = l == 0 ? used_next : nullptr;
-        const int extra = (l == 0 && k.commit_ovf) ? (int)S - 1 : -1;
-        if (l + 1 == h.nred) {
-            SRS_LAUNCH((k_slot_reduce<C, true>), (ceil_div((uint64_t)n_out * 4, 256), batch), (256), 0, stream, in, in_pb, used, (size_t)NBUCKET, extra,
-                       out, out_pb);
+        const bool quad = l + 1 == h.nred;
+        const dim3 grid(ceil_div(quad ? (uint64_t)n_out * 4 : (uint64_t)n_out, 256), batch);
+        if (l == 0) {
+            const uint8_t *used = used_next;
+            const int extra = k.commit_ovf ? (int)S - 1 : -1;
+            const auto reduce = quad ? &k_slot_reduce<C, true, xyzz29_t> : &k_slot_reduce<C, false, xyzz29_t>;
+            SRS_LAUNCH(reduce, (grid), (256), 0, stream, (const xyzz29_t *)k.slots, in_pb, used, (size_t)NBUCKET, extra, out, out_pb);
         } else {
-            SRS_LAUNCH((k_slot_reduce<C, false>), (ceil_div(n_out, 256), batch), (256), 0, stream, in, in_pb, used, (size_t)NBUCKET, extra, out,
-                       out_pb);
+            const auto reduce = quad ? &k_slot_reduce<C, true, xyzz_t> : &k_slot_reduce<C, false, xyzz_t>;
+            SRS_LAUNCH(reduce, (grid), (256), 0, stream, in, in_pb, (const uint8_t *)nullptr, (size_t)NBUCKET, -1, out, out_pb);
         }
         in = out;
         in_pb = out_pb;
diff --git a/sirius_amd/csrc/tuning.h b/sirius_amd/csrc/tuning.h
--- a/sirius_amd/csrc/tuning.h
+++ b/sirius_amd/csrc/tuning.h
@@ -20,6 +20,7 @@
     NO_JIT,
     MSM_COMPACT,
     PG_COMPAT_TREE,
+    MSM_SLOT_LEN,
     N_TUNABLES
 };
 
diff --git a/sirius_amd/csrc/tuning.hip b/sirius_amd/csrc/tuning.hip
--- a/sirius_amd/csrc/tuning.hip
+++ b/sirius_amd/csrc/tuning.hip
@@ -8,7 +8,7 @@
 
 static std::atomic<int64_t> g_val[N_TUNABLES];
 static const char *const kNames[N_TUNABLES] = {"msm_sort", "msm_l0", "msm_wide", "msm_wide_min", "msm_slots", "msm_slot_log", "msm_expect_ovf",
-                                               "msm_quad_max", "commit_chunks", "pg_f_eval", "pg_g_fft", "jit_always", "no_jit", "msm_compact", "pg_compat_tree"};
+                                               "msm_quad_max", "commit_chunks", "pg_f_eval", "pg_g_fft", "jit_always", "no_jit", "msm_compact", "pg_compat_tree", "msm_slot_len"};
 static struct Init {
     Init() { for (auto &v : g_val) v.store(UNSET, std::memory_order_relaxed); }
 } g_init;
```

Result: no change. 99.04 (-0.3%).
